# ktncktnc/diffusion-forcing-transformer

Hardware: AMD Instinct MI355X
Metric: denoised latent frames/sec, DFoT RE10K 8f & 200f rollout @1/2/4/8 GPU (higher is better)
Workload: dtype bf16

## Files before the change

### diffusion-forcing-transformer_amd/backbone.py

```python
from __future__ import annotations

import ctypes as C
import math
from typing import Dict, Optional, Sequence, Tuple

import torch
from torch import nn

from . import capi, ops


def _get(cfg, key, default=None):
    if isinstance(cfg, dict):
        return cfg.get(key, default)
    return getattr(cfg, key, default) if not hasattr(cfg, "get") else cfg.get(key, default)


class _Node(nn.Module):
    """Anonymous container so that dotted reference key names map onto a module tree."""


class UViT3DPose(nn.Module):
    def __init__(self, cfg, x_shape: Sequence[int], max_tokens: int, external_cond_dim: int = 0,
                 external_cond_type: str = "action", external_cond_num_classes: Optional[int] = None,
                 use_causal_mask: bool = False, **kwargs):
        super().__init__()
        block_types = list(_get(cfg, "block_types", ["ResBlock", "ResBlock", "TransformerBlock", "TransformerBlock"]))
        if block_types != ["ResBlock", "ResBlock", "TransformerBlock", "TransformerBlock"]:
            raise ValueError(f"unsupported block_types {block_types}")
        if _get(cfg, "pos_emb_type", "rope") != "rope":
            raise ValueError("only pos_emb_type='rope' is supported")
        if not _get(cfg, "use_fourier_noise_embedding", True):
            raise ValueError("only the Fourier noise-level embedding (continuous diffusion) is supported")
        cond = _get(cfg, "conditioning", None)
        cond_dim = _get(cond, "dim", None) if cond is not None else None
        self.cfg = cfg
        self.x_shape = tuple(x_shape)
        self.max_tokens = self.temporal_length = int(max_tokens)
        self.external_cond_dim = int(cond_dim or 180)
        self.use_causal_mask = use_causal_mask
        c = capi.UViTConfig()
        c.channels[:] = list(_get(cfg, "channels"))
        c.emb_channels = int(_get(cfg, "emb_channels"))
        c.num_updown_blocks[:] = list(_get(cfg, "num_updown_blocks"))
        c.num_mid_blocks = int(_get(cfg, "num_mid_blocks"))
        c.num_heads = int(_get(cfg, "num_heads"))
        c.in_channels = int(self.x_shape[0])
        c.resolution = int(self.x_shape[-1])
        c.max_tokens = self.max_tokens
        c.cond_dim = self.external_cond_dim
        c.noise_dim = 256
        c.rope_theta = 10000.0
        c.eps = 1e-6
        if int(_get(cfg, "patch_size", 2)) != 2:
            raise ValueError("only patch_size=2 is supported")
        self._ccfg = c
        self._handle = C.c_void_p()
        capi.check(capi.lib.dfot_uvit_create(C.byref(c), C.byref(self._handle)))
        self._names = []
        self._persistent_buffers = {"noise_level_pos_embedding.timesteps.freqs",
                                    "noise_level_pos_embedding.timesteps.phases"}
        shape = (C.c_int64 * 4)()
        ndim = C.c_int()
        for i in range(capi.lib.dfot_uvit_num_params(self._handle)):
            name = capi.lib.dfot_uvit_param_name(self._handle, i).decode()
            capi.check(capi.lib.dfot_uvit_param_shape(self._handle, i, shape, C.byref(ndim)))
            self._register(name, tuple(shape[k] for k in range(ndim.value)))
            self._names.append(name)
        self._synced: Optional[Tuple] = None
        self._reserved = 0
        self._op_key: Optional[int] = None
        self._cond_key = None
        self._cond_refs = None
        self._cond_gen = None
        self._cond_flag = None
        self.cond_cache_stats = {"builds": 0, "identity_hits": 0, "content_hits": 0}
        self._train_names = None
        self._trainer = None
        self._trainer_sig = None
        self.live_frames = None
        self.fresh_frames = None
        self._fresh_key = None
        self._train_stamp = 0
        self._dropout_generator: Optional[torch.Generator] = None

    def _register(self, name: str, shape: Tuple[int, ...]) -> None:
        *path, leaf = name.split(".")
        node: nn.Module = self
        for part in path:
            if part not in node._modules:
                node.add_module(part, _Node())
            node = node._modules[part]
        t = torch.zeros(shape, dtype=torch.float32)
        if name in self._persistent_buffers:
            node.register_buffer(leaf, t, persistent=True)
        else:
            node.register_parameter(leaf, nn.Parameter(t))

    def _tensors(self) -> Dict[str, torch.Tensor]:
        sd = dict(self.named_parameters())
        sd.update(dict(self.named_buffers()))
        return sd

    def reset_parameters(self, seed: int = 0) -> None:
        g = torch.Generator().manual_seed(seed)
        with torch.no_grad():
            for name, t in self._tensors().items():
                leaf = name.rsplit(".", 1)[-1]
                if leaf == "freqs":
                    t.copy_(2 * math.pi * torch.randn(t.shape, generator=g))
                elif leaf == "phases":
                    t.copy_(2 * math.pi * torch.rand(t.shape, generator=g))
                elif any(s in name for s in (".attn_out.", ".mlp_out.2.", ".out_rest.1.", "project_output")):
                    t.zero_()
                elif leaf == "bias":
                    t.zero_()
                elif t.ndim == 1:
                    t.fill_(1.0)
                else:
                    fan_in = math.prod(t.shape[1:])
                    bound = 1.0 / math.sqrt(fan_in)
                    t.copy_((torch.rand(t.shape, generator=g) * 2 - 1) * bound)

    def _signature(self) -> Tuple:
        return tuple((t.data_ptr(), t._version) for t in self._tensors().values())

    def sync_weights(self, force: bool = False) -> None:
        sig = self._signature()
        if not force and sig == self._synced:
            return
        tensors = self._tensors()
        s = capi.stream_ptr()
        for name in self._names:
            t = tensors[name]
            if not t.is_cuda:
                raise RuntimeError(f"parameter {name} is on {t.device}; move the module to the GPU first")
            src = t.detach().to(torch.float32).contiguous()
            shape = (C.c_int64 * src.ndim)(*src.shape)
            capi.check(capi.lib.dfot_uvit_load_weight(self._handle, name.encode(), capi.ptr(src), shape, src.ndim, s))
        capi.check(capi.lib.dfot_uvit_finalize(self._handle, s))
        self._synced = sig
        self.reserve_generation = getattr(self, "reserve_generation", 0) + 1

    def set_option(self, key: str, value: int) -> None:
        self.reserve_generation = getattr(self, "reserve_generation", 0) + 1
        capi.check(capi.lib.dfot_uvit_set_option(self._handle, key.encode(), int(value)))

    def query(self, key: str) -> float:
        self.sync_weights()
        val = C.c_double()
        capi.check(capi.lib.dfot_uvit_query(self._handle, key.encode(), C.byref(val)))
        return float(val.value)

    def attn_timing(self):
        tot, n = C.c_double(), C.c_int64()
        capi.check(capi.lib.dfot_uvit_attn_timing(self._handle, C.byref(tot), C.byref(n)))
        return tot.value, n.value

    def init_random(self, seed: int = 0, zero_init_scale: float = 0.3) -> None:
        g = torch.Generator().manual_seed(seed)
        with torch.no_grad():
            for name, t in self._tensors().items():
                leaf = name.rsplit(".", 1)[-1]
                if leaf == "freqs":
                    v = 2 * math.pi * torch.randn(t.shape, generator=g)
# ... 89 lines not shown
            out.append(eng.dx_in.to(grad_out.dtype))
        return out

    def _cond_content_equal(self, cond: torch.Tensor, mask: Optional[torch.Tensor]) -> bool:
        if self._cond_key is None or self._cond_refs is None:
            return False
        kept, kept_mask = self._cond_refs
        _, version, shape, synced, mask_key = self._cond_key
        if synced != self._synced or self._cond_gen != self.reserve_generation:
            return False
        if kept._version != version or (kept_mask is not None and kept_mask._version != mask_key[1]):
            return False
        for t in (cond, kept):
            if t.dtype != torch.float32 or not t.is_contiguous():
                return False
        if cond.device != kept.device or tuple(cond.shape) != shape:
            return False
        if (mask is None) != (kept_mask is None):
            return False
        if mask is not None and (mask.dtype != kept_mask.dtype or mask.shape != kept_mask.shape or mask.device != kept_mask.device
                                 or not mask.is_contiguous() or not kept_mask.is_contiguous()):
            return False
        if torch.cuda.is_current_stream_capturing():
            return False
        if self._cond_flag is None or self._cond_flag.device != cond.device:
            self._cond_flag = torch.zeros(1, dtype=torch.int32, device=cond.device)
        flag = self._cond_flag
        flag.zero_()
        s = capi.stream_ptr()
        capi.check(capi.lib.dfot_op_equal_bits(capi.ptr(kept), capi.ptr(cond), cond.numel() * cond.element_size(), capi.ptr(flag), s))
        if mask is not None:
            capi.check(capi.lib.dfot_op_equal_bits(capi.ptr(kept_mask), capi.ptr(mask), mask.numel() * mask.element_size(), capi.ptr(flag), s))
        return int(flag.item()) == 0

    def _forward_impl(self, x: torch.Tensor, noise_levels: torch.Tensor, external_cond: Optional[torch.Tensor] = None,
                      external_cond_mask: Optional[torch.Tensor] = None) -> torch.Tensor:
        assert x.shape[1] == self.temporal_length, (
            f"Temporal length of U-ViT is set to {self.temporal_length}, but input has temporal length {x.shape[1]}.")
        assert external_cond is not None, "External condition (camera pose) is required for U-ViT3DPose model."
        b = x.shape[0]
        if tuple(x.shape[2:]) != self.x_shape:
            raise ValueError(f"x has frame shape {tuple(x.shape[2:])}, expected {self.x_shape}")
        if tuple(external_cond.shape) != (b, self.temporal_length, self.external_cond_dim, *self.x_shape[1:]):
            raise ValueError(f"external_cond has shape {tuple(external_cond.shape)}")
        if external_cond_mask is not None:
            assert external_cond_mask.ndim == 1, "embedding mask should be of shape (B,)"
        if tuple(noise_levels.shape) != (b, self.temporal_length):
            raise ValueError(f"noise_levels has shape {tuple(noise_levels.shape)}, expected {(b, self.temporal_length)}")
        dev = next(self.parameters()).device
        if dev.type != "cuda":
            raise RuntimeError(f"the backbone's parameters are on {dev}; move the module to the GPU first (there is no CPU path)")
        capi.require_device(dev, x=x, noise_levels=noise_levels, external_cond=external_cond, external_cond_mask=external_cond_mask)
        self.sync_weights()
        self.reserve(b)
        xf = x.detach().to(torch.float32).contiguous()
        kf = noise_levels.detach().to(torch.float32).contiguous()
        key = (external_cond.data_ptr(), external_cond._version, tuple(external_cond.shape), self._synced,
               None if external_cond_mask is None else (external_cond_mask.data_ptr(), external_cond_mask._version))
        if key == self._cond_key:
            self.cond_cache_stats["identity_hits"] += 1
        else:
            if self._cond_content_equal(external_cond, external_cond_mask):
                self.cond_cache_stats["content_hits"] += 1
            else:
                cf = external_cond.detach().to(torch.float32).contiguous()
                mf = None if external_cond_mask is None else external_cond_mask.to(torch.uint8).contiguous()
                capi.check(capi.lib.dfot_uvit_set_conditions(self._handle, capi.ptr(cf, torch.float32, "external_cond"),
                                                             capi.ptr(mf, torch.uint8, "external_cond_mask"), b, capi.stream_ptr()))
                self.cond_cache_stats["builds"] += 1
            self._cond_key = key
            self._cond_refs = (external_cond, external_cond_mask)
            self._cond_gen = self.reserve_generation
        out = torch.empty_like(xf)
        live = self.live_frames
        if live is not None:
            if tuple(live.shape) != (b, self.temporal_length) or live.dtype != torch.uint8 or not live.is_contiguous():
                raise ValueError(f"live_frames must be a contiguous uint8 tensor of shape {(b, self.temporal_length)}")
            capi.require_device(dev, live_frames=live)
        fresh = self.fresh_frames
        if fresh is not None:
            if tuple(fresh.shape) != (b, self.temporal_length) or fresh.dtype != torch.uint8 or not fresh.is_contiguous():
                raise ValueError(f"fresh_frames must be a contiguous uint8 tensor of shape {(b, self.temporal_length)}")
            capi.require_device(dev, fresh_frames=fresh)
            if key != self._fresh_key:
                fresh = None
        capi.check(capi.lib.dfot_uvit_forward_cached_masks(self._handle, capi.ptr(xf, torch.float32, "x"),
                                                           capi.ptr(kf, torch.float32, "noise_levels"), capi.ptr(out), b,
                                                           capi.ptr(live, torch.uint8, "live_frames"),
                                                           capi.ptr(fresh, torch.uint8, "fresh_frames"), capi.stream_ptr()))
        self._fresh_key = key
        return out.to(x.dtype)

    def read_tap(self, name: str, channels: int, level: int, batch: int) -> torch.Tensor:
        r = self.x_shape[-1] // 2 // (2 ** level)
        out = torch.empty(batch * self.temporal_length, channels, r, r, device="cuda", dtype=torch.float32)
        capi.check(capi.lib.dfot_uvit_read_tap(self._handle, name.encode(), capi.ptr(out), out.numel(), capi.stream_ptr()))
        return out

    def __del__(self):
        try:
            if getattr(self, "_handle", None) and self._handle.value:
                capi.lib.dfot_uvit_destroy(self._handle)
                self._handle = C.c_void_p()
        except Exception:
            pass
```

### diffusion-forcing-transformer_amd/capi.py

```python
from __future__ import annotations

import ctypes as C
import os

_HERE = os.path.dirname(os.path.abspath(__file__))
LIB_PATH = os.environ.get("DFOT_LIB", os.path.join(_HERE, "libdfot_hip.so"))

OK, ERR_ARG, ERR_SHAPE, ERR_HIP, ERR_STATE, ERR_NAME = range(6)


class DfotError(RuntimeError):
    def __init__(self, code: int, message: str):
        super().__init__(f"libdfot_hip error {code}: {message}")
        self.code = code


class UViTConfig(C.Structure):
    _fields_ = [
        ("channels", C.c_int32 * 4), ("emb_channels", C.c_int32), ("num_updown_blocks", C.c_int32 * 3),
        ("num_mid_blocks", C.c_int32), ("num_heads", C.c_int32), ("in_channels", C.c_int32),
        ("resolution", C.c_int32), ("max_tokens", C.c_int32), ("cond_dim", C.c_int32), ("noise_dim", C.c_int32),
        ("rope_theta", C.c_float), ("eps", C.c_float),
    ]


class UViT3DConfig(C.Structure):
    _fields_ = UViTConfig._fields_ + [("cond_dropout", C.c_int32)]


class DiTConfig(C.Structure):
    _fields_ = [
        ("hidden_size", C.c_int32), ("depth", C.c_int32), ("num_heads", C.c_int32), ("patch_size", C.c_int32),
        ("in_channels", C.c_int32), ("height", C.c_int32), ("width", C.c_int32), ("max_tokens", C.c_int32),
        ("mlp_hidden", C.c_int32), ("noise_dim", C.c_int32), ("timesteps", C.c_int32),
        ("rope_theta", C.c_float), ("eps", C.c_float),
        ("variant", C.c_int32), ("embed_col_dim", C.c_int32), ("num_col_heads", C.c_int32), ("num_row_heads", C.c_int32),
        ("temporal_mlp_hidden", C.c_int32), ("use_bias", C.c_int32),
        ("cond_type", C.c_int32), ("cond_dim", C.c_int32), ("num_classes", C.c_int32), ("cond_dropout", C.c_int32),
        ("use_temporal_rope", C.c_int32),
    ]


class DiTConfigF(DiTConfig):
    _fields_ = [("fourier_noise", C.c_int32)]


class DiT1DConfig(C.Structure):
    _fields_ = [
        ("hidden", C.c_int32), ("depth", C.c_int32), ("heads", C.c_int32), ("mlp_hidden", C.c_int32), ("in_channels", C.c_int32),
        ("tokens_per_frame", C.c_int32), ("max_tokens", C.c_int32), ("timesteps", C.c_int32), ("causal", C.c_int32), ("eps", C.c_float),
    ]


COND_NONE, COND_ACTION, COND_LABEL = 0, 1, 2
ATTN_MAP_OFF, ATTN_MAP_FRAME, ATTN_MAP_FULL = -1, 0, 1


_P, _I, _L, _F = C.c_void_p, C.c_int, C.c_int64, C.c_float
_I32 = C.c_int32


class GemmDesc(C.Structure):
    _fields_ = [
        ("amode", _I32), ("epi", _I32), ("variant", _I32),
        ("A", _P), ("lda", _L), ("W", _P), ("ldw", _L),
        ("M", _I32), ("N", _I32), ("K", _I32), ("H", _I32), ("Wd", _I32), ("Cin", _I32),
        ("live", _P), ("bias", _P), ("bias_rows", _I32),
        ("out_f32", _P), ("out_bf16", _P), ("ldo", _L),
        ("resid", _P), ("resid_bf", _P),
        ("gate", _P), ("gate_index", _P), ("ldg", _L), ("gate_rows", _I32),
        ("act", _I32), ("pre_act", _P), ("raw", _P), ("ldraw", _L), ("tr_rows", _I32),
        ("gn_part", _P), ("gn_rows_per_bt", _I32), ("gn_cpg", _I32),
        ("out2", _P), ("ldo2", _L), ("split", _I32),
        ("q", _P), ("k", _P), ("v", _P),
        ("qw", _P), ("kw", _P), ("rope_cs", _P),
        ("heads", _I32), ("d", _I32), ("ntok", _I32), ("qscale", _F), ("dstride", _I32), ("eps", _F),
        ("ksplit", _I32), ("slice_stride", _L),
    ]


SIGNATURES = {
    "dfot_last_error": (C.c_char_p, []),
    "dfot_version": (_I, []),
    "dfot_uvit_create": (_I, [C.POINTER(UViTConfig), C.POINTER(_P)]),
    "dfot_uvit_destroy": (_I, [_P]),
    "dfot_uvit_num_params": (_I, [_P]),
    "dfot_uvit_param_name": (C.c_char_p, [_P, _I]),
    "dfot_uvit_param_shape": (_I, [_P, _I, C.POINTER(_L), C.POINTER(_I)]),
    "dfot_uvit_load_weight": (_I, [_P, C.c_char_p, _P, C.POINTER(_L), _I, _P]),
    "dfot_uvit_finalize": (_I, [_P, _P]),
    "dfot_uvit_reserve": (_I, [_P, _I]),
    "dfot_uvit_workspace_bytes": (C.c_size_t, [_P]),
    "dfot_uvit_set_option": (_I, [_P, C.c_char_p, _I]),
    "dfot_uvit_query": (_I, [_P, C.c_char_p, C.POINTER(C.c_double)]),
    "dfot_uvit_attn_timing": (_I, [_P, C.POINTER(C.c_double), C.POINTER(_L)]),
    "dfot_uvit_forward": (_I, [_P, _P, _P, _P, _P, _P, _I, _P]),
    "dfot_uvit_set_conditions": (_I, [_P, _P, _P, _I, _P]),
    "dfot_uvit_forward_cached": (_I, [_P, _P, _P, _P, _I, _P]),
    "dfot_uvit_forward_cached_live": (_I, [_P, _P, _P, _P, _I, _P, _P]),
    "dfot_uvit_forward_cached_masks": (_I, [_P, _P, _P, _P, _I, _P, _P, _P]),
    "dfot_uvit_read_tap": (_I, [_P, C.c_char_p, _P, C.c_size_t, _P]),
    "dfot_uvit3d_create": (_I, [C.POINTER(UViT3DConfig), C.POINTER(_P)]),
    "dfot_uvit3d_config_bytes": (_L, []),
    "dfot_uvit3d_forward": (_I, [_P, _P, _P, _P, _P, _P, _I, _P]),
    "dfot_uvit3d_forward_live": (_I, [_P, _P, _P, _P, _P, _P, _I, _P, _P]),
    "dfot_op_gn_film_silu": (_I, [_P, _P, _P, _P, _P, _P, _P, _P, _I, _I, _I, _I, _P]),
    "dfot_op_rms_film": (_I, [_P, _P, _P, _P, _P, _P, _L, _I, _I, _I, _F, _P]),
    "dfot_dit_create": (_I, [C.POINTER(DiTConfig), C.POINTER(_P)]),
    "dfot_dit_create_f": (_I, [C.POINTER(DiTConfigF), C.POINTER(_P)]),
    "dfot_dit_destroy": (_I, [_P]),
    "dfot_dit_num_params": (_I, [_P]),
    "dfot_dit_param_name": (C.c_char_p, [_P, _I]),
    "dfot_dit_param_shape": (_I, [_P, _I, C.POINTER(_L), C.POINTER(_I)]),
    "dfot_dit_load_weight": (_I, [_P, C.c_char_p, _P, C.POINTER(_L), _I, _P]),
    "dfot_dit_finalize": (_I, [_P, _P]),
    "dfot_dit_reserve": (_I, [_P, _I]),
    "dfot_dit_workspace_bytes": (C.c_size_t, [_P]),
    "dfot_dit_set_option": (_I, [_P, C.c_char_p, _I]),
    "dfot_dit_attn_timing": (_I, [_P, C.POINTER(C.c_double), C.POINTER(_L)]),
    "dfot_dit_forward": (_I, [_P, _P, _P, _P, _I, _I, _P]),
    "dfot_dit_forward_cond": (_I, [_P, _P, _P, _P, _P, _P, _P, _I, _I, _P]),
    "dfot_dit_forward_f": (_I, [_P, _P, _P, _P, _P, _P, _P, _I, _I, _P]),
    "dfot_dit_read_tap": (_I, [_P, C.c_char_p, _P, C.c_size_t, _P]),
    "dfot_dit_capture_attention": (_I, [_P, C.POINTER(_I32), _I, _I, C.c_size_t]),
    "dfot_dit_attention_map_shape": (_I, [_P, _I, C.POINTER(_L), C.POINTER(_I)]),
    "dfot_dit_read_attention_map": (_I, [_P, _I, _P, C.c_size_t, _P]),
    "dfot_dit_train_create": (_I, [C.POINTER(DiTConfig), C.POINTER(_P)]),
    "dfot_dit_train_create_f": (_I, [C.POINTER(DiTConfigF), C.POINTER(_P)]),
    "dfot_facmat_train_create": (_I, [C.POINTER(DiTConfigF), C.POINTER(_P)]),
    "dfot_facdit_train_create": (_I, [C.POINTER(DiTConfigF), C.POINTER(_P)]),
    "dfot_dit_train_destroy": (_I, [_P]),
    "dfot_dit_train_num_params": (_I, [_P]),
    "dfot_dit_train_param_name": (C.c_char_p, [_P, _I]),
    "dfot_dit_train_param_shape": (_I, [_P, _I, C.POINTER(_L), C.POINTER(_I)]),
    "dfot_dit_train_param_offset": (_L, [_P, _I]),
    "dfot_dit_train_total_numel": (_L, [_P]),
    "dfot_dit_train_workspace_bytes": (C.c_size_t, [_P]),
    "dfot_dit_train_attach": (_I, [_P, _P, _P]),
    "dfot_dit_train_reserve": (_I, [_P, _I]),
    "dfot_dit_train_sync_weights": (_I, [_P, _P]),
    "dfot_dit_train_forward": (_I, [_P, _P, _P, _P, _I, _I, _P]),
    "dfot_dit_train_forward_cond": (_I, [_P, _P, _P, _P, _P, _P, _P, _I, _I, _P]),
    "dfot_dit_train_load_buffer": (_I, [_P, C.c_char_p, _P, _L, _P]),
    "dfot_dit_train_forward_f": (_I, [_P, _P, _P, _P, _P, _P, _P, _I, _I, _P]),
    "dfot_dit_train_input_grad": (_I, [_P, _P, _P]),
    "dfot_dit_train_backward": (_I, [_P, _P, _P]),
    "dfot_vloss_grad": (_I, [_P] * 7 + [_I, _I, _L, _I, _P]),
    "dfot_sumsq": (_I, [_P, _L, _P, _P]),
    "dfot_adamw_step": (_I, [_P, _P, _P, _P, _L, _F, _F, _F, _F, _F, _I, _P, _F, _P, _F, _P]),
    "dfot_ray_encode": (_I, [_P, _P, _I, _I, _I, _P]),
    "dfot_ray_encode_normalized": (_I, [_P, _P, _I, _I, _I, _P]),
    "dfot_hg_prepare": (_I, [_P, _P, _P, _P, _P, _I, _I, _I, _L, _P]),
    "dfot_ddim_compose": (_I, [_P] * 11 + [_I, _I, _I, _L, _P]),
    "dfot_ddim_compose_tokw": (_I, [_P] * 11 + [_I, _I, _I, _L, _P]),
    "dfot_ddim_noise": (_I, [_P] * 5 + [_I, _I, _I, _L, _I, _P]),
    "dfot_vpred_loss": (_I, [_P] * 9 + [_I, _I, _L, _P]),
    "dfot_vpred_loss_scratch_floats": (_L, [_I, _I, _L]),
    "dfot_vspace_loss": (_I, [_P] * 9 + [_I, _I, _L, _P]),
    "dfot_op_gemm": (_I, [_P, _I, _P, _P, _P, _I, _I, _I, _I, _P]),
    "dfot_op_conv3x3": (_I, [_P, _P, _P, _P, _I, _I, _I, _I, _I, _I, _P]),
    "dfot_op_gemm_ex": (_I, [C.POINTER(GemmDesc), _P]),
    "dfot_op_gemm_desc_bytes": (_L, []),
    "dfot_op_attention": (_I, [_P, _P, _P, _P, _I, _I, _I, _I, _I, _I, _P]),
    "dfot_op_attention_padded": (_I, [_P, _P, _P, _P, _I, _I, _I, _I, _I, _P]),
    "dfot_op_attention_seq64": (_I, [_P, _P, _P, _P, _I, _I, _I, _I, _P]),
    "dfot_op_attention_temporal": (_I, [_P, _P, _P, _P, _I, _I, _I, _I, _I, _I, _P]),
    "dfot_op_attention_temporal_bwd": (_I, [_P, _P, _P, _P, _I, _P, _P, _P, _I, _I, _I, _I, _I, _P]),
    "dfot_op_matrix_attention_rope": (_I, [_P, _P, _P, _I, _I, _I, _I, _I, _I, _F, _P]),
    "dfot_op_matrix_attention_rope_bwd": (_I, [_P, _P, _P, _P, _I, _I, _I, _I, _I, _I, _F, _P]),
    "dfot_op_attention_map_workspace_bytes": (C.c_size_t, [_I, _I, _I, _I, _I]),
    "dfot_op_attention_map": (_I, [_P, _P, _P, _P, C.c_size_t, _I, _I, _I, _I, _I, _I, _P]),
    "dfot_op_attention_temporal_map": (_I, [_P, _P, _P, _P, C.c_size_t, _I, _I, _I, _I, _I, _P]),
    "dfot_op_matrix_attention_map": (_I, [_P, _P, _P, _I, _I, _I, _I, _I, _I, _F, _P]),
    "dfot_op_matrix_attention": (_I, [_P, _P, _I, _I, _I, _I, _I, _I, _F, _P]),
    "dfot_op_facmat_contract": (_I, [_P, _P, _P, _I, _I, _I, _I, _P]),
    "dfot_op_facmat_expand": (_I, [_P, _P, _P, _I, _I, _I, _I, _P]),
    "dfot_op_attention_bwd": (_I, [_P, _P, _P, _P, _P, _I, _P, _P, _P, _I, _I, _I, _I, _P]),
    "dfot_op_conv3x3_bwd": (_I, [_P, _P, _P, _P, _P, _P, _I, _I, _I, _I, _I, _P]),
    "dfot_op_conv3x3_bwd2": (_I, [_P, _P, _P, _P, _P, _P, _P, _I, _I, _I, _I, _I, _P]),
    "dfot_op_gn_silu_bwd": (_I, [_P, _P, _P, _P, _P, _F, _P, _P, _P, _P, _I, _I, _I, _P]),
    "dfot_op_rms_film_bwd": (_I, [_P, _P, _P, _P, _F, _P, _P, _P, _L, _I, _I, _P]),
    "dfot_op_rms_film_bwd_res": (_I, [_P, _P, _P, _P, _F, _P, _P, _P, _P, _P, _L, _I, _P]),
    "dfot_op_qknorm_rope_bwd": (_I, [_P, _I, _P, _P, _P, _P, _P, _P, _F, _P, _I, _P, _P, _L, _I, _I, _I, _P]),
# ... 140 lines not shown
```

### diffusion-forcing-transformer_amd/csrc/gemm.h

```cpp
#pragma once
#include "common.h"

namespace dfot {

enum AMode { A_DENSE = 0, A_CONV3 = 1, A_CONV3T = 2 };
enum Epi { E_F32 = 0, E_BF16 = 1, E_QKV = 2, E_QKV_DIT = 3 };

struct GemmArgs {
  const bf16* A = nullptr;
  long lda = 0;
  const bf16* W = nullptr;
  long ldw = 0;
  int M = 0, N = 0, K = 0;
  int H = 0, Wd = 0, Cin = 0;
  const bf16* zeros = nullptr;
  const uint8_t* live = nullptr;
  int To = 0, Tin = 0, Hin = 0, Win = 0;
  int cs = 1, ct = 1, ckt = 1;
  const float* bias = nullptr;
  float* out_f32 = nullptr;
  bf16* out_bf16 = nullptr;
  long ldo = 0;
  const float* resid = nullptr;
  const bf16* resid_bf = nullptr;
  const float* gate = nullptr;
  const int* gate_index = nullptr;
  long ldg = 0;
  int gate_rows = 0;
  int act = 0;
  bf16* pre_act = nullptr;
  bf16* raw = nullptr;
  long ldraw = 0;
  int bias_rows = 0;
  int tr_rows = 0;
  float* gn_part = nullptr;
  int gn_rows_per_bt = 0;
  int gn_cpg = 0;
  bf16* out2 = nullptr;
  long ldo2 = 0;
  int split = 0;
  bf16 *q = nullptr, *k = nullptr, *v = nullptr;
  const float *qw = nullptr, *kw = nullptr, *rope_cs = nullptr;
  int heads = 0, d = 0, ntok = 0;
  float qscale = 1.f;
  int dstride = 0;
  float eps = 1e-6f;
  int xcd = 1;
  int persist = 0;
  int ksplit = 1;
  long slice_stride = 0;
};

enum GemmVariant {
  GEMM_REGS_128 = 0,
  GEMM_DMA_128 = 1,
  GEMM_DMA_256x256 = 4,
  GEMM_DMA_512x128 = 6,
  GEMM_DMA_128_KS2 = 8,
  GEMM_DMA_256x192 = 9,
  GEMM_DMA_128x192 = 10,
  GEMM_DMA3_256x144 = 14,
  GEMM_AUTO = -1
};
int gemm_pick_variant(int amode, int m, int n, int k, bool plain_f32 = false);
int launch_gemm(int amode, int epi, int variant, const GemmArgs& g, hipStream_t stream);

}
```

### diffusion-forcing-transformer_amd/csrc/gemm.hip

```cpp
#include "gemm.h"
#include "dfot_hip.h"

namespace dfot {

constexpr int BK = 64;
constexpr int wave_cols(int bn) { return bn % 64 == 0 ? 64 : 48; }
constexpr int tile_threads(int bm, int bn, int wtm, int ks) { return (bm / wtm) * (bn / wave_cols(bn)) * 64 * ks; }
constexpr int EP_LD = 68;

template <int N>
__device__ __forceinline__ void wait_all_but() {
  static_assert(N == 2 || N == 4 || N == 6 || N == 8 || N == 12, "unexpected load count");
  if constexpr (N == 2) asm volatile("s_waitcnt vmcnt(2)\n\ts_barrier" ::: "memory");
  if constexpr (N == 4) asm volatile("s_waitcnt vmcnt(4)\n\ts_barrier" ::: "memory");
  if constexpr (N == 6) asm volatile("s_waitcnt vmcnt(6)\n\ts_barrier" ::: "memory");
  if constexpr (N == 8) asm volatile("s_waitcnt vmcnt(8)\n\ts_barrier" ::: "memory");
  if constexpr (N == 12) asm volatile("s_waitcnt vmcnt(12)\n\ts_barrier" ::: "memory");
}

__device__ __forceinline__ void wait_all_but_n(int n) {
  switch (n) {
    case 1: asm volatile("s_waitcnt vmcnt(1)\n\ts_barrier" ::: "memory"); break;
    case 2: asm volatile("s_waitcnt vmcnt(2)\n\ts_barrier" ::: "memory"); break;
    case 3: asm volatile("s_waitcnt vmcnt(3)\n\ts_barrier" ::: "memory"); break;
// ... 741 lines not shown
  constexpr int lds = stage_lds > ep_lds ? stage_lds : ep_lds;
  const int ksplit = (EPI == E_F32 && (AMODE == A_DENSE || g.slice_stride > 0) && g.ksplit > 1) ? g.ksplit : 1;
  const int tiles = (g.M / BM_T) * ((g.N + BN_T - 1) / BN_T) * ksplit;
  GemmArgs ga = g;
  ga.xcd = 1;
  ga.persist = 1;
  constexpr bool kPersistOK = KS == 1 && nthreads <= 768;
  if constexpr (kPersistOK) {
    if (ga.persist > 0 && ksplit == 1) {
      const int resident = 256 * (lds <= 80 * 1024 ? 2 : 1);
      if (tiles > resident) {
        auto kp = gemm_kernel_persistent<BM_T, BN_T, WTM, NST, AMODE, EPI, DMA, KS, BKT>;
        static bool pattr_set = false;
        if (!pattr_set) {
          DFOT_CHECK_HIP(hipFuncSetAttribute(reinterpret_cast<const void*>(kp), hipFuncAttributeMaxDynamicSharedMemorySize, lds));
          pattr_set = true;
        }
        hipLaunchKernelGGL(kp, dim3(resident), dim3(nthreads), lds, stream, ga, tiles);
        DFOT_CHECK_HIP(hipGetLastError());
        return DFOT_OK;
      }
    }
  }
  auto kern = gemm_kernel<BM_T, BN_T, WTM, NST, AMODE, EPI, DMA, KS, BKT>;
  static bool attr_set = false;
  if (!attr_set) {
    DFOT_CHECK_HIP(hipFuncSetAttribute(reinterpret_cast<const void*>(kern), hipFuncAttributeMaxDynamicSharedMemorySize, lds));
    attr_set = true;
  }
  hipLaunchKernelGGL(kern, dim3(tiles), dim3(nthreads), lds, stream, ga);
  DFOT_CHECK_HIP(hipGetLastError());
  return DFOT_OK;
}

template <int AMODE, int EPI>
static int launch_v(int variant, const GemmArgs& g, hipStream_t s) {
  switch (variant) {
    case GEMM_REGS_128:
      if constexpr (AMODE == A_CONV3T) break;
      else return launch_t<128, 128, 64, 2, AMODE, EPI, false>(g, s);
    case GEMM_DMA_128: return launch_t<128, 128, 64, 2, AMODE, EPI, true>(g, s);
    case GEMM_DMA_256x256: return launch_t<256, 256, 64, 2, AMODE, EPI, true>(g, s);
    case GEMM_DMA_512x128: return launch_t<512, 128, 64, 2, AMODE, EPI, true>(g, s);
    case GEMM_DMA_256x192:
      if constexpr (AMODE != A_DENSE) break;
      else return launch_t<256, 192, 64, 2, AMODE, EPI, true>(g, s);
    case GEMM_DMA3_256x144:
      if constexpr ((EPI != E_F32 && !(EPI == E_BF16 && AMODE == A_DENSE)) || AMODE == A_CONV3T) break;
      else {
        if (g.gn_part) break;
        return launch_t<256, 144, 64, 3, AMODE, EPI, true>(g, s);
      }
    case GEMM_DMA_128x192:
      if constexpr (AMODE != A_DENSE || EPI == E_QKV) break;
      else return launch_t<128, 192, 64, 2, AMODE, EPI, true>(g, s);
    case GEMM_DMA_128_KS2:
      if constexpr (EPI == E_QKV) break;
      else return launch_t<128, 128, 64, 2, AMODE, EPI, true, 2>(g, s);
  }
  set_error("gemm: unknown variant %d", variant);
  return DFOT_ERR_ARG;
}

int gemm_pick_variant(int amode, int m, int n, int k, bool plain_f32) {
  const long tiles = (long)(m / 256) * ((n + 255) / 256);
  if (m % 256 == 0 && n >= 192 && amode == A_DENSE) {
    auto util = [&](int bn) {
      const long t = (long)(m / 256) * ((n + bn - 1) / bn);
      return (double)m * n / ((double)((t + 255) / 256) * 256 * 256 * bn);
    };
    if (plain_f32 && n % 144 == 0 && k >= 2304 && (long)(m / 256) * (n / 144) >= 256 && util(144) > 1.1 * util(192) && util(144) > 1.1 * util(256))
      return GEMM_DMA3_256x144;
    if (util(192) > 1.05 * util(256) && (long)(m / 256) * ((n + 191) / 192) >= 160) return GEMM_DMA_256x192;
  }
  if (m % 256 == 0 && n >= 192 && tiles >= 160) return GEMM_DMA_256x256;
  if (m % 512 == 0 && n <= 128 && m / 512 >= 256) return GEMM_DMA_512x128;
  const long tiles128 = (long)(m / 128) * ((n + 127) / 128);
  if (tiles128 <= 256 && k >= 2048) return GEMM_DMA_128_KS2;
  return GEMM_DMA_128;
}

int launch_gemm(int amode, int epi, int variant, const GemmArgs& g, hipStream_t stream) {
  DFOT_REQUIRE(g.A && g.W, DFOT_ERR_ARG, "gemm: null operand");
  if (variant == GEMM_AUTO) variant = gemm_pick_variant(amode, g.M, g.N, g.K, epi == E_F32 && !g.gn_part);
  if (variant == GEMM_DMA_128_KS2 && epi == E_QKV) variant = GEMM_DMA_128;
  if (variant == GEMM_DMA_128x192 && epi == E_QKV) variant = GEMM_DMA_128;
  if (variant == GEMM_DMA_256x192 && epi == E_QKV && g.d != 64) variant = GEMM_DMA_256x256;
  const int bm = variant == GEMM_DMA_512x128 ? 512 : (variant == GEMM_DMA_256x256 || variant == GEMM_DMA_256x192 || variant == GEMM_DMA3_256x144) ? 256 : 128;
  DFOT_REQUIRE(g.M > 0 && g.M % bm == 0, DFOT_ERR_SHAPE, "gemm: M=%d must be a positive multiple of %d", g.M, bm);
  DFOT_REQUIRE(g.K > 0 && g.K % BK == 0, DFOT_ERR_SHAPE, "gemm: K=%d must be a positive multiple of %d", g.K, BK);
  DFOT_REQUIRE(g.N > 0 && g.N % (epi == E_F32 ? 4 : 8) == 0, DFOT_ERR_SHAPE, "gemm: N=%d must be a multiple of %d", g.N, epi == E_F32 ? 4 : 8);
  DFOT_REQUIRE((epi == E_QKV || epi == E_QKV_DIT || g.ldo % (epi == E_F32 ? 4 : 8) == 0) && (epi != E_QKV || (g.ldo2 % 8 == 0 && g.split % 64 == 0)),
               DFOT_ERR_SHAPE, "gemm: output row strides must be multiples of %d", epi == E_F32 ? 4 : 8);
  DFOT_REQUIRE(g.ldw == 0 || (amode == A_DENSE && g.ldw >= g.K && g.ldw % 8 == 0), DFOT_ERR_SHAPE, "gemm: ldw=%ld must be >= K and a multiple of 8 (dense A only)", g.ldw);
  if (amode == A_CONV3) {
    DFOT_REQUIRE(g.Cin % BK == 0 && g.K == 9 * g.Cin, DFOT_ERR_SHAPE, "conv3x3: Cin=%d must be a multiple of %d", g.Cin, BK);
    DFOT_REQUIRE(g.zeros != nullptr, DFOT_ERR_ARG, "conv3x3: zero page missing");
    DFOT_REQUIRE(g.H > 0 && g.Wd > 0 && g.M % (g.H * g.Wd) == 0, DFOT_ERR_SHAPE, "conv3x3: M=%d not a whole number of %dx%d images", g.M, g.H, g.Wd);
    DFOT_REQUIRE(!g.live || (g.H * g.Wd) % bm == 0, DFOT_ERR_SHAPE, "conv3x3: live-image flags need whole %d-row tiles per %dx%d image", bm, g.H, g.Wd);
  }
  if (amode == A_CONV3T) {
    DFOT_REQUIRE(epi == E_F32 && g.ksplit <= 1 && !g.live && !g.gate && !g.bias_rows, DFOT_ERR_ARG, "conv3t: plain fp32 epilogue only");
    DFOT_REQUIRE(g.Cin % BK == 0 && (g.ckt == 1 || g.ckt == 3) && g.K == g.ckt * 9 * g.Cin && (g.cs == 1 || g.cs == 2) && (g.ct == 1 || g.ct == 2),
                 DFOT_ERR_SHAPE, "conv3t: Cin=%d (multiple of %d), kt=%d in {1,3}, K=%d = kt*9*Cin, strides s=%d t=%d in {1,2}", g.Cin, BK, g.ckt, g.K,
                 g.cs, g.ct);
    DFOT_REQUIRE(g.zeros != nullptr, DFOT_ERR_ARG, "conv3t: zero page missing");
    DFOT_REQUIRE(g.H > 0 && g.Wd > 0 && g.To > 0 && g.Hin == g.cs * g.H && g.Win == g.cs * g.Wd && g.Tin >= 1 && g.ct * (g.To - 1) <= g.Tin - 1 &&
                     g.To == (g.Tin - 1) / g.ct + 1,
                 DFOT_ERR_SHAPE, "conv3t: input %dx%dx%d, output %dx%dx%d do not match strides s=%d t=%d", g.Tin, g.Hin, g.Win, g.To, g.H, g.Wd, g.cs, g.ct);
    DFOT_REQUIRE(g.M % (g.To * g.H * g.Wd) == 0, DFOT_ERR_SHAPE, "conv3t: M=%d not a whole number of %dx%dx%d videos", g.M, g.To, g.H, g.Wd);
    DFOT_REQUIRE((long)g.Tin * g.Hin * g.Win * g.Cin < (1L << 31), DFOT_ERR_SHAPE, "conv3t: one input video must hold < 2^31 elements");
  }
  if (epi == E_QKV) {
    DFOT_REQUIRE(g.q && g.k && g.v && g.qw && g.kw && g.rope_cs && (g.out2 || g.N == g.split), DFOT_ERR_ARG, "qkv epilogue: null pointer");
    DFOT_REQUIRE(!g.raw || (g.ldraw >= g.N && g.ldraw % 8 == 0), DFOT_ERR_SHAPE, "qkv epilogue: raw copy needs ldraw >= N, a multiple of 8");
    DFOT_REQUIRE((g.d == 64 || g.d == 128) && g.heads > 0 && g.split == 3 * g.heads * g.d && g.ntok > 0 && g.M % g.ntok == 0,
                 DFOT_ERR_SHAPE, "qkv epilogue: heads=%d d=%d split=%d ntok=%d M=%d", g.heads, g.d, g.split, g.ntok, g.M);
  }
  if (epi == E_QKV_DIT) {
    DFOT_REQUIRE(g.q && g.k && g.v, DFOT_ERR_ARG, "dit qkv epilogue: null pointer");
    DFOT_REQUIRE(g.d > 0 && g.d % 8 == 0 && g.dstride >= g.d && g.dstride % 8 == 0 && g.heads > 0 && g.N == 3 * g.heads * g.d &&
                     g.ntok > 0 && g.M % g.ntok == 0,
                 DFOT_ERR_SHAPE, "dit qkv epilogue: heads=%d d=%d dstride=%d ntok=%d M=%d N=%d", g.heads, g.d, g.dstride, g.ntok, g.M, g.N);
  }
  if (g.gate) {
    DFOT_REQUIRE(epi == E_F32 && g.gate_rows > 0 && g.M % g.gate_rows == 0 && g.ldg % 4 == 0, DFOT_ERR_SHAPE,
                 "gemm: gate needs the fp32 epilogue, gate_rows dividing M and ldg %% 4 == 0");
  }
  if (g.ksplit > 1 && g.slice_stride > 0)
    DFOT_REQUIRE(!g.bias && !g.resid, DFOT_ERR_ARG, "gemm: split-K into partial outputs takes no bias / residual");
  if (g.ksplit > 1)
    DFOT_REQUIRE(epi == E_F32 && (amode == A_DENSE || g.slice_stride > 0) && !g.bias_rows && (!g.resid || g.resid == g.out_f32) && !g.gate &&
                     !g.gn_part && g.K / BK >= 2 * g.ksplit, DFOT_ERR_ARG,
                 "gemm: split-K over workgroups needs the fp32 epilogue with an in-place residual (or none), no gate, and K >= %d", 2 * g.ksplit * BK);
  if (g.bias_rows) DFOT_REQUIRE((epi == E_F32 || epi == E_BF16) && g.bias, DFOT_ERR_ARG, "gemm: 2-D bias needs a plain epilogue");
  if (g.resid_bf)
    DFOT_REQUIRE(epi == E_BF16 && (amode == A_CONV3 || variant == GEMM_DMA3_256x144) && !g.resid, DFOT_ERR_ARG,
                 "gemm: a bf16 residual needs the bf16 epilogue of a convolution or of the 256x144 ring");
  if (g.tr_rows) {
    DFOT_REQUIRE(epi == E_BF16 && !g.bias && !g.act && !g.gn_part && g.tr_rows % 4 == 0 && g.M % g.tr_rows == 0 && amode == A_DENSE,
                 DFOT_ERR_ARG, "gemm: transposed store needs the plain bf16 epilogue and tr_rows %% 4 == 0 dividing M");
  }
  if (g.gn_part) {
    DFOT_REQUIRE(epi != E_QKV && epi != E_QKV_DIT && (g.gn_cpg == 4 || g.gn_cpg == 8) && g.N == 32 * g.gn_cpg && g.gn_rows_per_bt % 64 == 0 &&
                     g.gn_rows_per_bt % bm == 0,
                 DFOT_ERR_SHAPE, "gemm: fused GroupNorm statistics need N = 32 groups of 4 or 8 channels and whole images per tile");
  }
  if (amode == A_DENSE) {
    switch (epi) {
      case E_F32: return launch_v<A_DENSE, E_F32>(variant, g, stream);
      case E_BF16: return launch_v<A_DENSE, E_BF16>(variant, g, stream);
      case E_QKV: return launch_v<A_DENSE, E_QKV>(variant, g, stream);
      case E_QKV_DIT: return launch_v<A_DENSE, E_QKV_DIT>(variant, g, stream);
    }
  } else if (amode == A_CONV3) {
    switch (epi) {
      case E_F32: return launch_v<A_CONV3, E_F32>(variant, g, stream);
      case E_BF16: return launch_v<A_CONV3, E_BF16>(variant, g, stream);
    }
  } else if (amode == A_CONV3T && epi == E_F32) {
    return launch_v<A_CONV3T, E_F32>(variant, g, stream);
  }
  set_error("gemm: unsupported mode/epilogue combination %d/%d", amode, epi);
  return DFOT_ERR_ARG;
}

}
// ... 1 lines not shown
```

### diffusion-forcing-transformer_amd/csrc/kernels.h

```cpp
#pragma once
#include "common.h"

namespace dfot {

int launch_noise_emb(const float* k, const float* freqs, const float* phases, const float* w1, const float* b1,
                     const float* w2, const float* b2, float* hidden, float* out, int bt, int ndim, int e, hipStream_t s);
int launch_uvit3d_emb(const float* k, const float* freqs, const float* phases, const float* w1, const float* b1, const float* w2,
                      const float* b2, const float* cond, const uint8_t* cond_mask, const float* a_w1, const float* a_b1,
                      const float* a_w2, const float* a_b2, float* out, int bt, int ndim, int cdim, int e, int tokens, hipStream_t s);
int launch_embed_input(const float* x, const float* w, const float* b, float* out, int bt, int res, int cin, int c0,
                       hipStream_t s);
int launch_cond_repack(const float* cond, bf16* a, int bt, int res, int cdim, int kpad, hipStream_t s);
int launch_emb_pyramid(const bf16* emb0, bf16* emb1, bf16* emb2, bf16* emb3, int bt, int r0, int e, hipStream_t s);
int launch_project_output(const float* x0, const float* w, const float* b, float* out, int bt, int res, int c0, int cout,
                          hipStream_t s, const uint8_t* live = nullptr);
int launch_gn_partial_f32(const float* x, float* partial, int bt, int pixels, int c, hipStream_t s);
int launch_gn_partial_bf16(const bf16* x, float* partial, int bt, int pixels, int c, hipStream_t s);
int launch_gn_finalize(const float* partial, float* stats, int bt, int nblk, int pixels, int c, float eps, hipStream_t s);
int gn_partial_blocks(int pixels);
int launch_gn_apply_silu(const float* x, const float* stats, const float* gamma, const float* beta, bf16* out, int bt,
                         int pixels, int c, hipStream_t s, const uint8_t* live = nullptr);
struct FilmChunk {
  const bf16* w;
  const float* b;
  long out_off;
  int rows;
};
int launch_film_vec(const FilmChunk* table, int chunks, const float* nemb, float* sv, int bt, int e, hipStream_t s);
int launch_gn_film_silu(const bf16* h, const float* stats, const float* gamma, const float* beta, const bf16* fcache,
                        const float* sv, const uint8_t* cond_mask, bf16* out, int bt, int pixels, int c, int tokens,
                        hipStream_t s, const uint8_t* live = nullptr);
struct RmsPending {
  void* x;
  const float* bias;
  const float* s0;
  const float* s1;
  const float* s2;
};
int launch_rms_film(const float* x, const float* w, const bf16* fcache, const float* sv, const uint8_t* cond_mask, bf16* out,
                    long m, int c, int rows_per_bt, int tokens, float eps, hipStream_t s, const RmsPending* pend = nullptr);
int launch_rms_film_bf16(const bf16* x, const float* w, const bf16* fcache, const float* sv, const uint8_t* cond_mask, bf16* out,
                         long m, int c, int rows_per_bt, int tokens, float eps, hipStream_t s, const RmsPending* pend = nullptr);

int launch_pool2_bf16(const float* x, bf16* out, int bt, int h, int w, int c, hipStream_t s);
int launch_pool2_bf16_bf16in(const bf16* x, bf16* out, int bt, int h, int w, int c, hipStream_t s);
int launch_sub_bf16_bf16in(const bf16* a, const float* b, bf16* out, long n, hipStream_t s, const uint8_t* live = nullptr, long frame_elems = 0);
int launch_upsample_add_bf16(const float* t, const bf16* skip, bf16* out, int bt, int h, int w, int c, hipStream_t s, const uint8_t* live = nullptr);
int launch_gn_apply_silu_bf16in(const bf16* x, const float* stats, const float* gamma, const float* beta, bf16* out, int bt, int pixels, int c,
                                hipStream_t s, const uint8_t* live = nullptr);
int launch_embed_input_bf16(const float* x, const float* w, const float* b, bf16* out, int bt, int res, int cin, int c0, hipStream_t s);
int launch_project_output_bf16(const bf16* x0, const float* w, const float* b, float* out, int bt, int res, int c0, int cout, hipStream_t s,
                               const uint8_t* live = nullptr);
int launch_sub_bf16(const float* a, const float* b, bf16* out, long n, hipStream_t s, const uint8_t* live = nullptr, long frame_elems = 0);
int launch_upsample_add(const float* t, const float* skip, float* out, int bt, int h, int w, int c, hipStream_t s, const uint8_t* live = nullptr);
int launch_ray_encode(const float* poses, float* out, int b, int t, int res, int normalized, hipStream_t s);
int launch_hg_prepare(const float* x, const float* noise, const float* qa, const float* qb, float* x_in, int batch,
                      int nfe, int tokens, long f, hipStream_t s);
int launch_ddim_compose(const float* x, const float* x_in, const float* v, const float* sa, const float* s1,
                        const float* an, const float* cn, const float* keep, const float* weight, const uint8_t* gen,
                        float* x_next, int batch, int nfe, int tokens, long f, bool weight_per_token, hipStream_t s);
int launch_ddim_noise(const float* noise, const float* sigma, const float* weight, const uint8_t* gen, float* x_next, int batch, int nfe,
                      int tokens, long f, bool weight_per_token, hipStream_t s);
int vloss_chunks(long f);
int launch_vloss(const float* x, const float* noise, const float* v, const float* a, const float* sg, const float* w,
                 float* x_pred, float* partial, float* loss, int batch, int tokens, long f, bool vspace, hipStream_t s);
int launch_wgrad_nt(const bf16* a, long lda, const bf16* b, long ldb, float* out, int m, int n, long rows, int slices, hipStream_t s, int img_h = 0,
                    int img_w = 0, int sdy = 0, int sdx = 0, int all_taps = 0);
struct WgradPlan {
  int form, slices;
};
WgradPlan wgrad_plan(int m, int n, long rows, long max_slices);
int launch_wgrad_conv_taps(const bf16* dy, const bf16* x, float* out, int co, int ci, long pix, int slices, int img_h, int img_w, hipStream_t s);
int wgrad_conv_tiles(int co, int ci, int* target);
int launch_wgrad_nt_plan(const bf16* a, long lda, const bf16* b, long ldb, float* out, int m, int n, long rows, WgradPlan plan, hipStream_t s);
int launch_vloss_grad(const float* x, const float* noise, const float* v, const float* a, const float* sg, const float* coef, float* dv,
                      int batch, int tokens, long f, bool vspace, hipStream_t s);
int launch_sumsq(const float* x, long n, float* out, hipStream_t s);
int launch_adamw(float* p, const float* g, float* m, float* v, long n, float lr, float b1, float b2, float eps, float wd, int step,
                 const float* sumsq, float max_norm, float* ema, float ema_decay, hipStream_t s);
int launch_f32_to_bf16(const float* src, bf16* dst, long n, hipStream_t s);
int launch_bf16_to_f32(const bf16* src, float* dst, long n, hipStream_t s);
int launch_equal_bits(const void* a, const void* b, long bytes, int* differs, hipStream_t s);
int launch_pack_rows(const float* src, bf16* dst, const int* map, int rows, int k, int kpad, long ldd, int col0,
                     hipStream_t s);
int launch_pack_conv3(const float* src, bf16* dst, int co, int ci, hipStream_t s);
int launch_gather_f32(const float* src, float* dst, const int* map, int n, hipStream_t s);
int launch_nhwc_to_nchw(const float* src, float* dst, int bt, int p, int c, hipStream_t s);
int launch_bf16_nhwc_to_nchw(const bf16* src, float* dst, int bt, int p, int c, hipStream_t s);

struct AttnScratch {
  float* p = nullptr;
  size_t bytes = 0;
};
int launch_attention(const bf16* q, const bf16* k, const bf16* v, bf16* o, long ldo, int batch, int heads, int n, int d,
                     int variant, hipStream_t stream, AttnScratch* scratch = nullptr);
int launch_attention_v3(const bf16* q, const bf16* k, const bf16* v, bf16* o, long ldo, int batch, int heads, int n, bool nomax,
                        hipStream_t stream, AttnScratch* scratch = nullptr);
bool attention_v5_applies(int n, int d, float score_bound);
int launch_attention_v5(const bf16* q, const bf16* k, const bf16* v, bf16* o, long ldo, int batch, int heads, int n, hipStream_t stream,
                        AttnScratch* scratch = nullptr, float* lse = nullptr);
bool attention_ks_applies(int batch, int heads, int n, int d);
size_t attention_ks_scratch_bytes(int batch, int heads, int n, int d);
int launch_attention_ks(const bf16* q, const bf16* k, const bf16* v, bf16* o, long ldo, int batch, int heads, int n, hipStream_t stream,
                        AttnScratch* scratch = nullptr);
int attention_dstride(int d);
int launch_attention_padded(const bf16* q, const bf16* k, const bf16* v, bf16* o, long ldo, int batch, int heads, int n, int d,
                            hipStream_t stream, float* lse = nullptr);
int launch_attention_seq64(const bf16* q, const bf16* k, const bf16* v, bf16* o, long ldo, int nseq, int heads, int d, hipStream_t stream);
int launch_attention_frame_causal(const bf16* q, const bf16* k, const bf16* v, bf16* o, long ldo, int batch, int heads, int n, int frame_len,
                                  int d, hipStream_t stream);
int launch_attention_temporal(const bf16* q, const bf16* k, const bf16* v, bf16* o, long ldo, int batch, int tokens, int patches, int heads,
                              int d, hipStream_t s);
int launch_attention_temporal_bwd(const bf16* q, const bf16* k, const bf16* v, const bf16* d_o, long ldo, bf16* dq, bf16* dk, bf16* dv,
                                  int batch, int tokens, int patches, int heads, int d, hipStream_t s);
int launch_matrix_attn_rope(const bf16* z, bf16* o, const float* rope_cs, int batch, int L, int E, int h, int cc, int rr, float scale,
                            hipStream_t s);
int launch_matrix_attn_rope_bwd(const bf16* z, const bf16* d_o, const float* rope_cs, bf16* dz, int batch, int L, int E, int h, int cc, int rr,
                                float scale, hipStream_t s);
int launch_facmat_contract(const bf16* m, const bf16* u, bf16* w, int frames, int P, int h, int E, hipStream_t s);
int launch_facmat_expand(const bf16* o, const bf16* u, bf16* sp, int frames, int P, int h, int E, hipStream_t s);
size_t attention_map_part_floats(int batch, int heads, int n, int tokens);
int launch_attention_map(const bf16* q, const bf16* k, float* out, float* part, bool full, int batch, int heads, int n, int tokens, int d,
                         hipStream_t s);
size_t attention_temporal_map_part_floats(int batch, int heads, int tokens, int patches);
int launch_attention_temporal_map(const bf16* q, const bf16* k, float* out, float* part, int batch, int tokens, int patches, int heads, int d,
                                  hipStream_t s);
int launch_matrix_attn_map(const bf16* z, const float* rope_cs, float* out, int batch, int L, int E, int h, int cc, int rr, float scale,
                           hipStream_t s);
struct AttnSplit {
  int tiles, full, rem, nsplit;
  int slots;
};
AttnSplit attn_plan_split(int batch, int heads, int n, int qrows, int wgs_per_cu);
size_t attn_partial_bytes(const AttnSplit& sp, int qrows, int dcols);
size_t attention_scratch_bytes(int batch, int heads, int n, int d);
int attn_partials(const AttnSplit& sp, int qrows, int dcols, float** po, float** pml, AttnScratch* scratch);
int attn_launch_merge(const AttnSplit& sp, int qrows, int dcols, const float* po, const float* pml, bf16* o, long ldo, int n, int heads,
                      hipStream_t stream, float* lse = nullptr);
int launch_attention_bwd_delta(const bf16* o, const bf16* d_o, long ldo, float* delta, int batch, int heads, int n, int d, hipStream_t s);
int launch_attention_bwd(const bf16* q, const bf16* k, const bf16* v, const bf16* d_o, long ldo, const float* l2, const float* delta,
                         bf16* dq, bf16* dk, bf16* dv, int batch, int heads, int n, int d, hipStream_t s);

}
```

### diffusion-forcing-transformer_amd/csrc/kernels.hip

```cpp
#include "kernels.h"
#include "dfot_hip.h"

namespace dfot {

typedef __attribute__((ext_vector_type(4))) float float4v;
typedef __attribute__((ext_vector_type(2))) float float2v;

__device__ __forceinline__ float wave_sum(float v) {
#pragma unroll
  for (int o = 32; o > 0; o >>= 1) v += __shfl_xor(v, o);
  return v;
}

template <bool FOURIER>
__global__ __launch_bounds__(256) void noise_mlp_kernel(const float* __restrict__ in, const float* __restrict__ freqs,
                                                        const float* __restrict__ phases, const float* __restrict__ w,
                                                        const float* __restrict__ b, float* __restrict__ out, int kdim,
                                                        int e) {
  const int lane = threadIdx.x & 63, wave = threadIdx.x >> 6;
  const int row = blockIdx.x * 4 + wave;
  const int bt = blockIdx.y;
  if (row >= e) return;
  float acc = 0.f;
  for (int i = lane; i < kdim; i += 64) {
// ... 1441 lines not shown
  if (!part) DFOT_CHECK_HIP(hipMalloc(&part, SUMSQ_BLOCKS * sizeof(float)));
  hipLaunchKernelGGL(sumsq_partial_kernel, dim3(SUMSQ_BLOCKS), dim3(256), 0, s, x, n, part);
  hipLaunchKernelGGL(sumsq_final_kernel, dim3(1), dim3(256), 0, s, part, out);
  DFOT_CHECK_HIP(hipGetLastError());
  return DFOT_OK;
}

__global__ void adamw_kernel(float* __restrict__ p, const float* __restrict__ g, float* __restrict__ m, float* __restrict__ v, long n,
                             float lr, float b1, float b2, float eps, float wd, float c1, float c2, const float* __restrict__ sumsq,
                             float max_norm, float* __restrict__ ema, float ema_decay) {
  const long i = (long)blockIdx.x * blockDim.x + threadIdx.x;
  if (i >= n) return;
  float clip = 1.f;
  if (sumsq) clip = fminf(1.f, max_norm / (sqrtf(*sumsq) + 1e-6f));
  const float gv = g[i] * clip;
  const float mv = b1 * m[i] + (1.f - b1) * gv;
  const float vv = b2 * v[i] + (1.f - b2) * gv * gv;
  m[i] = mv;
  v[i] = vv;
  const float pv = p[i] * (1.f - lr * wd);
  const float pn = pv - (lr / c1) * mv / (sqrtf(vv) / sqrtf(c2) + eps);
  p[i] = pn;
  if (ema) ema[i] = ema_decay * ema[i] + (1.f - ema_decay) * pn;
}
int launch_adamw(float* p, const float* g, float* m, float* v, long n, float lr, float b1, float b2, float eps, float wd, int step,
                 const float* sumsq, float max_norm, float* ema, float ema_decay, hipStream_t s) {
  DFOT_REQUIRE(step >= 1, DFOT_ERR_ARG, "adamw: step counts from 1");
  const float c1 = (float)(1.0 - pow((double)b1, (double)step)), c2 = (float)(1.0 - pow((double)b2, (double)step));
  hipLaunchKernelGGL(adamw_kernel, dim3(cdiv(n, 256)), dim3(256), 0, s, p, g, m, v, n, lr, b1, b2, eps, wd, c1, c2, sumsq, max_norm, ema, ema_decay);
  DFOT_CHECK_HIP(hipGetLastError());
  return DFOT_OK;
}

typedef __attribute__((ext_vector_type(4))) unsigned int uint4v;
__device__ __forceinline__ unsigned int bits_differ(uint4v x, uint4v y) {
  const uint4v d = x ^ y;
  return d[0] | d[1] | d[2] | d[3];
}
__device__ __forceinline__ unsigned int bits_differ(unsigned int x, unsigned int y) { return x ^ y; }
__device__ __forceinline__ unsigned int bits_differ(uint8_t x, uint8_t y) { return (unsigned int)(x ^ y); }

constexpr int EQ_BLOCK = 256, EQ_MAX_GRID = 2048;

template <typename T>
__global__ __launch_bounds__(EQ_BLOCK) void equal_bits_kernel(const T* __restrict__ a, const T* __restrict__ b, long n, int rest,
                                                              int* __restrict__ differs) {
  const long stride = (long)gridDim.x * EQ_BLOCK;
  long i = (long)blockIdx.x * EQ_BLOCK + threadIdx.x;
  unsigned int acc = 0;
  for (; i + 3 * stride < n; i += 4 * stride) {
    const T a0 = a[i], a1 = a[i + stride], a2 = a[i + 2 * stride], a3 = a[i + 3 * stride];
    const T b0 = b[i], b1 = b[i + stride], b2 = b[i + 2 * stride], b3 = b[i + 3 * stride];
    acc |= bits_differ(a0, b0) | bits_differ(a1, b1) | bits_differ(a2, b2) | bits_differ(a3, b3);
  }
  for (; i < n; i += stride) acc |= bits_differ(a[i], b[i]);
  if (blockIdx.x == 0 && (int)threadIdx.x < rest) {
    const uint8_t* ta = reinterpret_cast<const uint8_t*>(a + n);
    const uint8_t* tb = reinterpret_cast<const uint8_t*>(b + n);
    acc |= bits_differ(ta[threadIdx.x], tb[threadIdx.x]);
  }
  if (acc) *differs = 1;
}

template <typename T>
static int launch_equal_bits_t(const void* a, const void* b, long bytes, int* differs, hipStream_t s) {
  const long n = bytes / (long)sizeof(T);
  const int rest = (int)(bytes - n * (long)sizeof(T));
  const int grid = n ? (int)(cdiv(n, EQ_BLOCK) < EQ_MAX_GRID ? cdiv(n, EQ_BLOCK) : EQ_MAX_GRID) : 1;
  hipLaunchKernelGGL(equal_bits_kernel<T>, dim3(grid), dim3(EQ_BLOCK), 0, s, (const T*)a, (const T*)b, n, rest, differs);
  DFOT_CHECK_HIP(hipGetLastError());
  return DFOT_OK;
}

int launch_equal_bits(const void* a, const void* b, long bytes, int* differs, hipStream_t s) {
  DFOT_REQUIRE(differs && ((uintptr_t)differs & 3) == 0, DFOT_ERR_ARG, "equal_bits: the flag is null or not 4-byte aligned");
  DFOT_REQUIRE(bytes >= 0, DFOT_ERR_ARG, "equal_bits: negative length %ld", bytes);
  if (bytes == 0) return DFOT_OK;
  DFOT_REQUIRE(a && b, DFOT_ERR_ARG, "equal_bits: null buffer");
  const uintptr_t al = (uintptr_t)a | (uintptr_t)b;
  if ((al & 15) == 0) return launch_equal_bits_t<uint4v>(a, b, bytes, differs, s);
  if ((al & 3) == 0) return launch_equal_bits_t<unsigned int>(a, b, bytes, differs, s);
  return launch_equal_bits_t<uint8_t>(a, b, bytes, differs, s);
}
}

extern "C" int dfot_op_equal_bits(const void* a, const void* b, int64_t bytes, int32_t* differs, void* stream) {
  return dfot::launch_equal_bits(a, b, (long)bytes, differs, (hipStream_t)stream);
}
```

### diffusion-forcing-transformer_amd/csrc/uvit.hip

```cpp
#include <algorithm>
#include <cmath>
#include <cstdarg>
#include <cstdlib>
#include <cstring>
#include <functional>
#include <map>
#include <string>
#include <vector>

#include "dfot_hip.h"
#include "gemm.h"
#include "kernels.h"

namespace dfot {

static thread_local char g_err[1024] = "";
void set_error(const char* fmt, ...) {
  va_list ap;
  va_start(ap, fmt);
  vsnprintf(g_err, sizeof(g_err), fmt, ap);
  va_end(ap);
}
const char* get_error() { return g_err; }

// ... 256 lines not shown
    bf16* pw = h->pose_w;
    const int k = c.cond_dim * 4, kp = h->kpose;
    add_param(h, "external_cond_embedding.patch_embedder.proj.weight", {e, c.cond_dim, 2, 2},
              [=](const float* src, hipStream_t s) { return launch_pack_rows(src, pw, nullptr, e, k, kp, kp, 0, s); });
    if ((rc = add_f32(h, "external_cond_embedding.patch_embedder.proj.bias", {e}, &h->pose_b))) return rc;
  }
  if ((rc = add_f32(h, "embed_input.proj.weight", {h->ch[0], c.in_channels, 2, 2}, &h->ein_w))) return rc;
  if ((rc = add_f32(h, "embed_input.proj.bias", {h->ch[0]}, &h->ein_b))) return rc;
  if ((rc = add_f32(h, "project_output.proj.weight", {h->ch[0], c.in_channels, 2, 2}, &h->pout_w))) return rc;
  if ((rc = add_f32(h, "project_output.proj.bias", {c.in_channels}, &h->pout_b))) return rc;

  for (int l = 0; l < 3; ++l) {
    const int n = c.num_updown_blocks[l];
    const std::string pre = "down_blocks." + std::to_string(l) + ".";
    if (l < 2) {
      h->down_res[l].resize(n);
      for (int i = 0; i < n; ++i)
        if ((rc = add_res_block(h, pre + std::to_string(i), h->ch[l], &h->down_res[l][i]))) return rc;
    } else {
      h->down_tr.resize(n);
      for (int i = 0; i < n; ++i)
        if ((rc = add_tr_block(h, pre + std::to_string(i), l, &h->down_tr[i]))) return rc;
    }
    if ((rc = add_conv(h, pre + std::to_string(n) + ".conv", h->ch[l], h->ch[l + 1], &h->down_conv[l]))) return rc;
  }
  auto add_mid = [&]() -> int {
    h->mid_tr.resize(c.num_mid_blocks);
    for (int i = 0; i < c.num_mid_blocks; ++i)
      if ((rc = add_tr_block(h, "mid_blocks." + std::to_string(i), 3, &h->mid_tr[i]))) return rc;
    return DFOT_OK;
  };
  if (!h->posefree && (rc = add_mid())) return rc;
  for (int j = 0; j < 3; ++j) {
    const int l = 2 - j;
    const int n = c.num_updown_blocks[l];
    const std::string pre = "up_blocks." + std::to_string(j) + ".";
    if ((rc = add_conv(h, pre + "0.conv", h->ch[l + 1], h->ch[l], &h->up_conv[l]))) return rc;
    if (l < 2) {
      h->up_res[l].resize(n);
      for (int i = 0; i < n; ++i)
        if ((rc = add_res_block(h, pre + std::to_string(i + 1), h->ch[l], &h->up_res[l][i]))) return rc;
    } else {
      h->up_tr.resize(n);
      for (int i = 0; i < n; ++i)
        if ((rc = add_tr_block(h, pre + std::to_string(i + 1), l, &h->up_tr[i]))) return rc;
    }
  }
  if (h->posefree && (rc = add_mid())) return rc;
  return DFOT_OK;
}

static int build_rope(dfot_uvit_s* h, int lvl) {
  const int d = h->ch[lvl] / h->heads, half = d / 2;
  const int q = half / 3, rem = half % 3;
  int parts[3] = {q, q, q};
  if (rem == 1) parts[0] = q + 1;
  if (rem == 2) parts[1] = parts[2] = q + 1;
  const int rr = h->r[lvl], n = h->T * rr * rr;
  std::vector<float> cs((size_t)n * half * 2);
  for (int tok = 0; tok < n; ++tok) {
    const int pos[3] = {tok / (rr * rr), (tok / rr) % rr, tok % rr};
    int pair = 0;
    for (int ax = 0; ax < 3; ++ax) {
      const int dim = 2 * parts[ax];
      for (int j = 0; j < parts[ax]; ++j, ++pair) {
        const float inv = 1.0f / powf(h->cfg.rope_theta, (float)(2 * j) / (float)dim);
        const float ang = (float)pos[ax] * inv;
        cs[((size_t)tok * half + pair) * 2 + 0] = cosf(ang);
        cs[((size_t)tok * half + pair) * 2 + 1] = sinf(ang);
      }
    }
  }
  int rc = dev_alloc(h, &h->rope_cs[lvl], cs.size());
  if (rc) return rc;
  DFOT_CHECK_HIP(hipMemcpy(h->rope_cs[lvl], cs.data(), cs.size() * sizeof(float), hipMemcpyHostToDevice));
  return DFOT_OK;
}

__global__ void add_vec_kernel(const float* a, const float* b, float* o, int n) {
  const int i = blockIdx.x * blockDim.x + threadIdx.x;
  if (i < n) o[i] = a[i] + b[i];
}

static int run_res_block(dfot_uvit_s* h, const ResW& w, int lvl, int bt, hipStream_t s, const uint8_t* live = nullptr) {
  const int c = w.c, rr = h->r[lvl], pix = rr * rr;
  const int m = bt * pix;
  const int slots = pix / 64;
  bf16* xb = h->XB[lvl];
  int rc = 0;
  if (!h->xin_bf[lvl]) {
    if ((rc = launch_f32_to_bf16(h->xin[lvl], xb, (long)m * c, s))) return rc;
    h->xin_bf[lvl] = true;
  }
  if (h->gn1_nblk == 0) {
    if ((rc = launch_gn_partial_bf16(xb, h->gn_partial, bt, pix, c, s))) return rc;
    h->gn1_nblk = gn_partial_blocks(pix);
  }
  if ((rc = launch_gn_finalize(h->gn_partial, h->gn_stats, bt, h->gn1_nblk, pix, c, h->cfg.eps, s))) return rc;
  h->gn1_nblk = 0;
  if ((rc = launch_gn_apply_silu_bf16in(xb, h->gn_stats, w.g1, w.be1, h->s1, bt, pix, c, s, live))) return rc;
  GemmArgs g;
  g.A = h->s1; g.W = w.w1; g.M = m; g.N = c; g.K = 9 * c; g.H = rr; g.Wd = rr; g.Cin = c; g.zeros = h->zeros;
  g.bias = w.bias1; g.out_bf16 = h->hbf; g.ldo = c; g.live = live;
  g.gn_part = h->gn_partial2; g.gn_rows_per_bt = pix; g.gn_cpg = c / 32;
  if ((rc = launch_gemm(A_CONV3, E_BF16, h->gemm_variant, g, s))) return rc;
  if ((rc = launch_gn_finalize(h->gn_partial2, h->gn_stats, bt, slots, pix, c, h->cfg.eps, s))) return rc;
  if ((rc = launch_gn_film_silu(h->hbf, h->gn_stats, w.g2, w.be2, w.fcache, h->sv + w.sv_off,
                                h->have_mask ? h->cond_mask : nullptr, h->s1, bt, pix, c, h->T, s, live)))
    return rc;
  GemmArgs o;
  o.A = h->s1; o.W = w.w2; o.M = m; o.N = c; o.K = 9 * c; o.H = rr; o.Wd = rr; o.Cin = c; o.zeros = h->zeros;
  o.bias = w.bias2; o.out_bf16 = xb; o.ldo = c; o.live = live;
  o.resid_bf = xb;
  o.gn_part = h->gn_partial; o.gn_rows_per_bt = pix; o.gn_cpg = c / 32;
  if ((rc = launch_gemm(A_CONV3, E_BF16, h->gemm_variant, o, s))) return rc;
  h->xin_bf[lvl] = true;
  h->gn1_nblk = slots;
  return DFOT_OK;
}

__global__ void out_reduce_kernel(bf16* x, const float* __restrict__ bias, const float* __restrict__ s0, const float* __restrict__ s1,
                                  const float* __restrict__ s2, long total4, int cq) {
  typedef __attribute__((ext_vector_type(4))) float f4;
  const long i = (long)blockIdx.x * blockDim.x + threadIdx.x;
  if (i >= total4) return;
  f4 b = reinterpret_cast<const f4*>(bias)[i % cq] + reinterpret_cast<const f4*>(s0)[i] + reinterpret_cast<const f4*>(s1)[i];
  if (s2) b += reinterpret_cast<const f4*>(s2)[i];
  const bf16x4 xv = reinterpret_cast<const bf16x4*>(x)[i];
  reinterpret_cast<bf16x4*>(x)[i] = bf16x4{f2bf(bf2f(xv[0]) + b[0]), f2bf(bf2f(xv[1]) + b[1]), f2bf(bf2f(xv[2]) + b[2]), f2bf(bf2f(xv[3]) + b[3])};
}
__global__ void add_f32_into_bf16_kernel(bf16* x, const float* __restrict__ y, long total4) {
  typedef __attribute__((ext_vector_type(4))) float f4;
  const long i = (long)blockIdx.x * blockDim.x + threadIdx.x;
  if (i >= total4) return;
  const f4 b = reinterpret_cast<const f4*>(y)[i];
  const bf16x4 xv = reinterpret_cast<const bf16x4*>(x)[i];
  reinterpret_cast<bf16x4*>(x)[i] = bf16x4{f2bf(bf2f(xv[0]) + b[0]), f2bf(bf2f(xv[1]) + b[1]), f2bf(bf2f(xv[2]) + b[2]), f2bf(bf2f(xv[3]) + b[3])};
}

static void swap_out_part(dfot_uvit_s* h) { h->pend_part = h->out_part; }

static int flush_pending(dfot_uvit_s* h, hipStream_t s) {
  if (!h->pend_bias) return DFOT_OK;
  const long total4 = h->pend_m * h->pend_c / 4;
  hipLaunchKernelGGL(out_reduce_kernel, dim3(cdiv(total4, 256)), dim3(256), 0, s, h->XB[h->pend_lvl], h->pend_bias, h->pend_part,
                     h->pend_part + h->pend_m * h->pend_c, h->pend_slices == 3 ? h->pend_part + 2 * h->pend_m * h->pend_c : nullptr, total4,
                     h->pend_c / 4);
  h->pend_bias = nullptr;
  DFOT_CHECK_HIP(hipGetLastError());
  return DFOT_OK;
}

static int run_tr_block(dfot_uvit_s* h, const TrW& w, int lvl, int batch, hipStream_t s) {
  const int c = w.c, rr = h->r[lvl], n = h->T * rr * rr, d = c / h->heads;
  const int m = batch * n;
  bf16* xb = h->XB[lvl];
  int rc = 0;
  if (h->pend_bias && (h->pend_lvl != lvl || h->pend_m != m || h->pend_c != c) && (rc = flush_pending(h, s))) return rc;
  if (!h->xin_bf[lvl]) {
    if ((rc = launch_f32_to_bf16(h->xin[lvl], xb, (long)m * c, s))) return rc;
    h->xin_bf[lvl] = true;
  }
  RmsPending pend{xb, h->pend_bias, h->pend_part, h->pend_part + (long)m * c, h->pend_slices == 3 ? h->pend_part + 2L * m * c : nullptr};
  if ((rc = launch_rms_film_bf16(xb, w.nw, w.fcache, h->sv + w.sv_off, h->have_mask ? h->cond_mask : nullptr, h->s1, m, c, rr * rr, h->T,
                                 h->cfg.eps, s, h->pend_bias ? &pend : nullptr)))
    return rc;
  h->pend_bias = nullptr;
  GemmArgs p;
  p.A = h->s1; p.lda = c; p.W = w.w_fused; p.M = m; p.N = 7 * c; p.K = c; p.bias = w.b_fused;
  p.out2 = h->cat + c; p.ldo2 = 5 * c; p.split = 3 * c;
  p.q = h->q; p.k = h->k; p.v = h->v; p.qw = w.qw; p.kw = w.kw; p.rope_cs = h->rope_cs[lvl]; p.heads = h->heads; p.d = d;
  p.ntok = n; p.qscale = 1.4426950408889634f / sqrtf((float)d); p.eps = h->cfg.eps;
  if ((rc = launch_gemm(A_DENSE, E_QKV, h->gemm_variant, p, s))) return rc;
  const bool timed = h->time_attn && lvl == 2 && h->ev_used < h->ev_start.size();
  if (timed) DFOT_CHECK_HIP(hipEventRecord(h->ev_start[h->ev_used], s));
  int av = h->attn_variant;
  if (av == 2 && d == 64 && n % 256 == 0) av = (attention_v5_applies(n, d, w.score_bound) && !h->attn_force_safe) ? 14 : 5;
  if ((rc = launch_attention(h->q, h->k, h->v, h->cat, 5 * c, batch, h->heads, n, d, av, s, &h->attn_scratch))) return rc;
  if (timed) DFOT_CHECK_HIP(hipEventRecord(h->ev_stop[h->ev_used++], s));
  GemmArgs o;
  o.A = h->cat; o.lda = 5 * c; o.W = w.w_out; o.M = m; o.N = c; o.K = 5 * c; o.bias = w.b_out; o.ldo = c;
  if (h->gemm_variant == GEMM_AUTO && h->out_part && (size_t)2 * m * c <= h->out_part_elems && m % 256 == 0 && c % 144 == 0 &&
      (long)(m / 256) * (c / 144) * 2 <= 256 && (5 * c / 64) >= 8) {
    GemmArgs p2 = o;
    p2.bias = nullptr; p2.out_f32 = h->out_part; p2.ksplit = 2; p2.slice_stride = (long)m * c;
    if ((rc = launch_gemm(A_DENSE, E_F32, GEMM_DMA3_256x144, p2, s))) return rc;
    h->pend_bias = w.b_out;
    h->pend_lvl = lvl; h->pend_m = m; h->pend_c = c; h->pend_slices = 2;
    swap_out_part(h);
    return DFOT_OK;
  }
  if (h->gemm_variant == GEMM_AUTO && c % 144 == 0 && m % 256 == 0 && (long)(m / 256) * ((c + 191) / 192) < 256 &&
      (long)(m / 256) * (c / 144) >= 200 && (long)(m / 256) * (c / 144) <= 256) {
    o.out_bf16 = xb;
    o.resid_bf = xb;
    return launch_gemm(A_DENSE, E_BF16, GEMM_DMA3_256x144, o, s);
  }
  o.out_f32 = h->X[lvl];
  if ((rc = launch_gemm(A_DENSE, E_F32, h->gemm_variant, o, s))) return rc;
  hipLaunchKernelGGL(add_f32_into_bf16_kernel, dim3(cdiv((long)m * c / 4, 256)), dim3(256), 0, s, xb, h->X[lvl], (long)m * c / 4);
  DFOT_CHECK_HIP(hipGetLastError());
  return DFOT_OK;
}


__global__ void slab_reduce_kernel(float* __restrict__ out, const float* __restrict__ bias, const float* __restrict__ slabs, int nslab, long stride4,
                                   long total4, int cq, const uint8_t* __restrict__ live, unsigned img4) {
  typedef __attribute__((ext_vector_type(4))) float f4;
  const long i = (long)blockIdx.x * blockDim.x + threadIdx.x;
  if (i >= total4) return;
  if (live && !live[(unsigned)i / img4]) return;
  f4 v = reinterpret_cast<const f4*>(bias)[i % cq];
  for (int sl = 0; sl < nslab; ++sl) v += reinterpret_cast<const f4*>(slabs)[sl * stride4 + i];
  reinterpret_cast<f4*>(out)[i] = v;
}

static int conv_between_levels(dfot_uvit_s* h, GemmArgs g, hipStream_t s) {
  const long px = (long)g.H * g.Wd;
  if (h->gemm_variant == GEMM_AUTO && h->out_part && !g.gn_part && g.M % 256 == 0 && px % 256 == 0 && (g.N % 144 == 0 || g.N == 256) &&
      (long)g.M * g.N < (1L << 31)) {
    const int bn = g.N % 144 == 0 ? 144 : 256;
    const int variant = bn == 144 ? GEMM_DMA3_256x144 : GEMM_DMA_256x256;
    const int tiles = (g.M / 256) * (g.N / bn);
    int ks = 1;
    while (tiles * ks * 2 <= 256 && g.K / 64 / (ks * 2) >= 16) ks *= 2;
    if (tiles * ks >= 192 && tiles * ks <= 256) {
      if (ks == 1) return launch_gemm(A_CONV3, E_F32, variant, g, s);
      if ((size_t)ks * g.M * g.N <= h->out_part_elems) {
        GemmArgs p = g;
        float* out = g.out_f32;
        const float* bias = g.bias;
        p.bias = nullptr; p.resid = nullptr; p.out_f32 = h->out_part; p.ksplit = ks; p.slice_stride = (long)g.M * g.N;
        int rc = launch_gemm(A_CONV3, E_F32, variant, p, s);
        if (rc) return rc;
        const long total4 = (long)g.M * g.N / 4;
        hipLaunchKernelGGL(slab_reduce_kernel, dim3(cdiv(total4, 256)), dim3(256), 0, s, out, bias, h->out_part, ks, total4, total4, g.N / 4, g.live,
                           (unsigned)(px * g.N / 4));
        DFOT_CHECK_HIP(hipGetLastError());
        return DFOT_OK;
      }
    }
  }
  return launch_gemm(A_CONV3, E_F32, h->gemm_variant, g, s);
}

static int run_down(dfot_uvit_s* h, int l, int bt, hipStream_t s, const uint8_t* live = nullptr) {
  const int rr = h->r[l], cin = h->ch[l], cout = h->ch[l + 1];
  int rc = 0;
  if ((rc = h->xin_bf[l] ? launch_pool2_bf16_bf16in(h->XB[l], h->s1, bt, rr, rr, cin, s) : launch_pool2_bf16(h->xin[l], h->s1, bt, rr, rr, cin, s)))
    return rc;
  GemmArgs g;
  g.A = h->s1; g.W = h->down_conv[l].w; g.M = bt * (rr / 2) * (rr / 2); g.N = cout; g.K = 9 * cin; g.H = rr / 2; g.Wd = rr / 2;
  g.Cin = cin; g.zeros = h->zeros; g.bias = h->down_conv[l].b; g.out_f32 = h->HSA[l]; g.ldo = cout;
  g.live = live;
  const bool next_is_res = l + 1 < 2;
  if (next_is_res) {
    g.gn_part = h->gn_partial; g.gn_rows_per_bt = (rr / 2) * (rr / 2); g.gn_cpg = cout / 32;
  }
  if ((rc = conv_between_levels(h, g, s))) return rc;
  h->gn1_nblk = next_is_res ? g.gn_rows_per_bt / 64 : 0;
  h->xin[l + 1] = h->HSA[l];
  h->xin_bf[l + 1] = false;
  return DFOT_OK;
}

static int run_up(dfot_uvit_s* h, int l, int bt, hipStream_t s, const uint8_t* live = nullptr) {
  const int rr = h->r[l + 1], cin = h->ch[l + 1], cout = h->ch[l];
  const long n_in = (long)bt * rr * rr * cin;
  int rc = 0;
  if ((rc = h->xin_bf[l + 1] ? launch_sub_bf16_bf16in(h->XB[l + 1], h->HSA[l], h->s1, n_in, s, live, (long)rr * rr * cin)
                             : launch_sub_bf16(h->xin[l + 1], h->HSA[l], h->s1, n_in, s, live, (long)rr * rr * cin)))
    return rc;
  GemmArgs g;
  g.A = h->s1; g.W = h->up_conv[l].w; g.M = bt * rr * rr; g.N = cout; g.K = 9 * cin; g.H = rr; g.Wd = rr; g.Cin = cin;
  g.zeros = h->zeros; g.bias = h->up_conv[l].b; g.out_f32 = h->tmp; g.ldo = cout;
  if (live && (rr * rr) % 256 == 0 && h->gemm_variant == GEMM_AUTO) g.live = live;
  if ((rc = conv_between_levels(h, g, s))) return rc;
  h->gn1_nblk = 0;
  if (!h->xin_bf[l]) {
    set_error("run_up: level %d stream is not in its bf16 buffer", l);
    return DFOT_ERR_STATE;
  }
  return launch_upsample_add_bf16(h->tmp, h->XB[l], h->XB[l], bt, rr, rr, cout, s, live);
}

}

static int forward_from_emb(dfot_uvit_s* h, const float* x, float* out, int batch, const uint8_t* live_frames, const uint8_t* fresh_frames,
                            hipStream_t s);

extern "C" {

const char* dfot_last_error(void) { return get_error(); }
int dfot_version(void) { return 1; }

int dfot_uvit_create(const dfot_uvit_config* cfg, dfot_uvit_t* out) {
  DFOT_REQUIRE(cfg && out, DFOT_ERR_ARG, "dfot_uvit_create: null argument");
  DFOT_REQUIRE(cfg->resolution % 16 == 0 && cfg->resolution >= 32, DFOT_ERR_SHAPE, "resolution %d must be a multiple of 16", cfg->resolution);
  DFOT_REQUIRE(cfg->emb_channels % 64 == 0, DFOT_ERR_SHAPE, "emb_channels %d must be a multiple of 64", cfg->emb_channels);
  DFOT_REQUIRE(cfg->in_channels <= 3 && cfg->cond_dim % 20 == 0, DFOT_ERR_SHAPE, "in_channels %d / cond_dim %d unsupported", cfg->in_channels, cfg->cond_dim);
  for (int l = 0; l < 4; ++l)
    DFOT_REQUIRE(cfg->channels[l] % 64 == 0, DFOT_ERR_SHAPE, "channels[%d]=%d must be a multiple of 64", l, cfg->channels[l]);
  DFOT_REQUIRE(cfg->channels[0] % 128 == 0 && cfg->channels[1] % 128 == 0, DFOT_ERR_SHAPE, "ResBlock channels must be multiples of 128");
  for (int l = 2; l < 4; ++l) {
    const int d = cfg->channels[l] / cfg->num_heads;
    DFOT_REQUIRE(d * cfg->num_heads == cfg->channels[l] && (d == 64 || d == 128), DFOT_ERR_SHAPE,
                 "level %d head dim %d must be 64 or 128", l, d);
  }
  const int r3 = cfg->resolution / 16;
  DFOT_REQUIRE((cfg->max_tokens * r3 * r3) % 128 == 0, DFOT_ERR_SHAPE, "tokens at the coarsest level (%d) must be a multiple of 128", cfg->max_tokens * r3 * r3);
  auto* h = new dfot_uvit_s();
  h->cfg = *cfg;
  int rc = build(h);
  if (rc) {
    dfot_uvit_destroy(h);
    return rc;
  }
  *out = h;
  return DFOT_OK;
}

int dfot_uvit_destroy(dfot_uvit_t h) {
  if (!h) return DFOT_OK;
  for (void* p : h->owned) (void)hipFree(p);
  for (void* p : h->ws_owned) (void)hipFree(p);
  for (hipEvent_t e : h->ev_start) (void)hipEventDestroy(e);
  for (hipEvent_t e : h->ev_stop) (void)hipEventDestroy(e);
  delete h;
  return DFOT_OK;
}

int dfot_uvit3d_create(const dfot_uvit3d_config* cfg, dfot_uvit_t* out) {
  DFOT_REQUIRE(cfg && out, DFOT_ERR_ARG, "dfot_uvit3d_create: null argument");
  DFOT_REQUIRE(cfg->resolution % 16 == 0 && cfg->resolution >= 32, DFOT_ERR_SHAPE, "resolution %d must be a multiple of 16", cfg->resolution);
  DFOT_REQUIRE(cfg->emb_channels % 64 == 0 && cfg->emb_channels <= 1024, DFOT_ERR_SHAPE,
               "emb_channels %d must be a multiple of 64 and at most 1024", cfg->emb_channels);
  DFOT_REQUIRE(cfg->in_channels >= 1 && cfg->in_channels <= 3, DFOT_ERR_SHAPE, "in_channels %d unsupported (1 .. 3)", cfg->in_channels);
  DFOT_REQUIRE(cfg->cond_dim >= 0 && cfg->cond_dim <= 1024, DFOT_ERR_SHAPE, "cond_dim %d unsupported: the action embedding takes 0 (none) .. 1024 values", cfg->cond_dim);
  DFOT_REQUIRE(cfg->noise_dim > 0 && cfg->noise_dim <= 1024, DFOT_ERR_SHAPE, "noise_dim %d must be 1 .. 1024", cfg->noise_dim);
  for (int l = 0; l < 4; ++l)
    DFOT_REQUIRE(cfg->channels[l] > 0 && cfg->channels[l] % 64 == 0, DFOT_ERR_SHAPE, "channels[%d]=%d must be a multiple of 64", l, cfg->channels[l]);
  DFOT_REQUIRE(cfg->channels[0] % 128 == 0 && cfg->channels[1] % 128 == 0, DFOT_ERR_SHAPE, "ResBlock channels must be multiples of 128");
  DFOT_REQUIRE(cfg->num_heads > 0 && cfg->max_tokens > 0 && cfg->num_mid_blocks >= 0, DFOT_ERR_SHAPE, "num_heads / max_tokens must be positive");
  for (int l = 2; l < 4; ++l) {
    const int d = cfg->channels[l] / cfg->num_heads;
    DFOT_REQUIRE(d * cfg->num_heads == cfg->channels[l] && (d == 64 || d == 128), DFOT_ERR_SHAPE,
                 "level %d head dim %d must be 64 or 128 (channels %d / num_heads %d)", l, d, cfg->channels[l], cfg->num_heads);
  }
  const int r3 = cfg->resolution / 16;
  DFOT_REQUIRE((cfg->max_tokens * r3 * r3) % 128 == 0, DFOT_ERR_SHAPE, "tokens at the coarsest level (%d) must be a multiple of 128", cfg->max_tokens * r3 * r3);
  auto* h = new dfot_uvit_s();
  dfot_uvit_config& c = h->cfg;
  for (int l = 0; l < 4; ++l) c.channels[l] = cfg->channels[l];
  for (int l = 0; l < 3; ++l) c.num_updown_blocks[l] = cfg->num_updown_blocks[l];
  c.emb_channels = cfg->emb_channels; c.num_mid_blocks = cfg->num_mid_blocks; c.num_heads = cfg->num_heads;
  c.in_channels = cfg->in_channels; c.resolution = cfg->resolution; c.max_tokens = cfg->max_tokens;
  c.cond_dim = 0;
  c.noise_dim = cfg->noise_dim; c.rope_theta = cfg->rope_theta; c.eps = cfg->eps;
  h->posefree = true;
  h->act_dim = cfg->cond_dim;
  h->act_dropout = cfg->cond_dim > 0 && cfg->cond_dropout != 0;
  int rc = build(h);
  if (rc) {
    dfot_uvit_destroy(h);
    return rc;
  }
  *out = h;
  return DFOT_OK;
}
int64_t dfot_uvit3d_config_bytes(void) { return (int64_t)sizeof(dfot_uvit3d_config); }

int dfot_uvit_num_params(dfot_uvit_t h) { return h ? (int)h->params.size() : 0; }
// ... 173 lines not shown
    h->ev_used = 0;
    while ((int)h->ev_start.size() < value) {
      hipEvent_t a, b;
      DFOT_CHECK_HIP(hipEventCreate(&a));
      DFOT_CHECK_HIP(hipEventCreate(&b));
      h->ev_start.push_back(a);
      h->ev_stop.push_back(b);
    }
  }
  else {
    set_error("set_option: unknown key '%s'", key);
    return DFOT_ERR_ARG;
  }
  return DFOT_OK;
}

int dfot_uvit_query(dfot_uvit_t h, const char* key, double* value) {
  DFOT_REQUIRE(h && key && value, DFOT_ERR_ARG, "query: null argument");
  DFOT_REQUIRE(h->finalized, DFOT_ERR_STATE, "query: weights not finalized");
  float bound = 0.f;
  for (const TrW& w : h->down_tr) bound = fmaxf(bound, w.score_bound);
  for (const TrW& w : h->up_tr) bound = fmaxf(bound, w.score_bound);
  if (!strcmp(key, "score_bound_l2")) *value = bound;
  else if (!strcmp(key, "attn_kernel_l2")) *value = (bound < 64.0f && !h->attn_force_safe) ? 14 : 5;
  else if (!strcmp(key, "cond_builds")) *value = (double)h->cond_builds;
  else {
    set_error("query: unknown key '%s'", key);
    return DFOT_ERR_ARG;
  }
  return DFOT_OK;
}

int dfot_uvit_set_conditions(dfot_uvit_t h, const float* external_cond, const uint8_t* external_cond_mask, int batch,
                             void* stream) {
  DFOT_REQUIRE(h, DFOT_ERR_ARG, "set_conditions: null handle");
  DFOT_REQUIRE(!h->posefree, DFOT_ERR_STATE, "set_conditions: a pose-free handle (dfot_uvit3d_create) has no pose caches; call dfot_uvit3d_forward");
  DFOT_REQUIRE(external_cond != nullptr, DFOT_ERR_ARG, "External condition (camera pose) is required for U-ViT3DPose model.");
  DFOT_REQUIRE(h->finalized, DFOT_ERR_STATE, "set_conditions: weights not finalized");
  DFOT_REQUIRE(batch > 0 && batch <= h->max_batch, DFOT_ERR_STATE, "set_conditions: batch %d exceeds reserved %d", batch, h->max_batch);
  hipStream_t s = (hipStream_t)stream;
  const dfot_uvit_config& c = h->cfg;
  const int bt = batch * h->T, e = h->E;
  int rc = 0;
  h->cond_batch = 0;
  ++h->cond_builds;
  if ((rc = launch_cond_repack(external_cond, h->acond, bt, c.resolution, c.cond_dim, h->kpose, s))) return rc;
  {
    GemmArgs g;
    g.A = h->acond; g.lda = h->kpose; g.W = h->pose_w; g.M = bt * h->r[0] * h->r[0]; g.N = e; g.K = h->kpose;
    g.bias = h->pose_b; g.out_bf16 = h->emb[0]; g.ldo = e;
    if ((rc = launch_gemm(A_DENSE, E_BF16, h->gemm_variant, g, s))) return rc;
  }
  if ((rc = launch_emb_pyramid(h->emb[0], h->emb[1], h->emb[2], h->emb[3], bt, h->r[0], e, s))) return rc;
  auto fill = [&](bf16* fcache, const bf16* wf, int cc, int lvl) -> int {
    GemmArgs g;
    g.A = h->emb[lvl]; g.lda = e; g.W = wf; g.M = bt * h->r[lvl] * h->r[lvl]; g.N = 2 * cc; g.K = e;
    g.out_bf16 = fcache; g.ldo = 2 * cc;
    return launch_gemm(A_DENSE, E_BF16, h->gemm_variant, g, s);
  };
  for (int l = 0; l < 2; ++l) {
    for (ResW& w : h->down_res[l]) if ((rc = fill(w.fcache, w.w_film, w.c, l))) return rc;
    for (ResW& w : h->up_res[l]) if ((rc = fill(w.fcache, w.w_film, w.c, l))) return rc;
  }
  for (TrW& w : h->down_tr) if ((rc = fill(w.fcache, w.w_film, w.c, 2))) return rc;
  for (TrW& w : h->up_tr) if ((rc = fill(w.fcache, w.w_film, w.c, 2))) return rc;
  for (TrW& w : h->mid_tr) if ((rc = fill(w.fcache, w.w_film, w.c, 3))) return rc;
  h->have_mask = external_cond_mask != nullptr;
  if (h->have_mask) DFOT_CHECK_HIP(hipMemcpyAsync(h->cond_mask, external_cond_mask, batch, hipMemcpyDeviceToDevice, s));
  h->cond_batch = batch;
  return DFOT_OK;
}

int dfot_uvit_forward_cached(dfot_uvit_t h, const float* x, const float* noise_levels, float* out, int batch, void* stream) {
  return dfot_uvit_forward_cached_live(h, x, noise_levels, out, batch, nullptr, stream);
}

int dfot_uvit_forward_cached_live(dfot_uvit_t h, const float* x, const float* noise_levels, float* out, int batch, const uint8_t* live_frames,
                                  void* stream) {
  return dfot_uvit_forward_cached_masks(h, x, noise_levels, out, batch, live_frames, nullptr, stream);
}

int dfot_uvit_forward_cached_masks(dfot_uvit_t h, const float* x, const float* noise_levels, float* out, int batch, const uint8_t* live_frames,
                                   const uint8_t* fresh_frames, void* stream) {
  DFOT_REQUIRE(h && x && noise_levels && out, DFOT_ERR_ARG, "forward: null argument");
  DFOT_REQUIRE(!fresh_frames || h->last_batch == batch, DFOT_ERR_STATE,
               "forward: frozen frames need the previous forward of this handle to have run the same batch (%d, now %d)", h->last_batch, batch);
  DFOT_REQUIRE(!fresh_frames || live_frames, DFOT_ERR_ARG, "forward: frozen frames must also be dead frames (live_frames is null)");
  DFOT_REQUIRE(!h->posefree, DFOT_ERR_STATE, "forward_cached: a pose-free handle (dfot_uvit3d_create) runs through dfot_uvit3d_forward");
  DFOT_REQUIRE(h->finalized, DFOT_ERR_STATE, "forward: weights not finalized");
  DFOT_REQUIRE(batch > 0 && batch == h->cond_batch, DFOT_ERR_STATE,
               "forward_cached: batch %d does not match the cached conditions (%d)", batch, h->cond_batch);
  hipStream_t s = (hipStream_t)stream;
  const dfot_uvit_config& c = h->cfg;
  const int bt = batch * h->T, e = h->E;
  int rc = 0;
  if ((rc = launch_noise_emb(noise_levels, h->ne_freqs, h->ne_phases, h->ne_w1, h->ne_b1, h->ne_w2, h->ne_b2, h->nhid,
                             h->nemb, bt, c.noise_dim, e, s)))
    return rc;
  return forward_from_emb(h, x, out, batch, live_frames, fresh_frames, s);
}

}

static int forward_from_emb(dfot_uvit_s* h, const float* x, float* out, int batch, const uint8_t* live_frames, const uint8_t* fresh_frames,
                            hipStream_t s) {
  const dfot_uvit_config& c = h->cfg;
  const int bt = batch * h->T, e = h->E;
  int rc = 0;
  if ((rc = launch_film_vec(h->film_table, h->film_chunks, h->nemb, h->sv, bt, e, s))) return rc;
  if ((rc = launch_embed_input_bf16(x, h->ein_w, h->ein_b, h->XB[0], bt, c.resolution, c.in_channels, h->ch[0], s))) return rc;
  h->gn1_nblk = 0;
  for (int l = 0; l < 4; ++l) h->xin[l] = h->X[l];
  h->xin_bf[0] = true;
  h->xin_bf[1] = h->xin_bf[2] = h->xin_bf[3] = false;

  if (fresh_frames && (h->gemm_variant != GEMM_AUTO || (h->r[2] * h->r[2]) % 512 != 0)) fresh_frames = nullptr;
  for (int l = 0; l < 2; ++l) {
    for (const ResW& w : h->down_res[l])
      if ((rc = run_res_block(h, w, l, bt, s, fresh_frames))) return rc;
    if ((rc = run_down(h, l, bt, s, fresh_frames))) return rc;
  }
  h->pend_bias = nullptr;
  for (const TrW& w : h->down_tr)
    if ((rc = run_tr_block(h, w, 2, batch, s))) return rc;
  if ((rc = flush_pending(h, s))) return rc;
  if ((rc = run_down(h, 2, bt, s))) return rc;
  for (const TrW& w : h->mid_tr)
    if ((rc = run_tr_block(h, w, 3, batch, s))) return rc;
  if ((rc = flush_pending(h, s))) return rc;
  if ((rc = run_up(h, 2, bt, s))) return rc;
  for (const TrW& w : h->up_tr)
    if ((rc = run_tr_block(h, w, 2, batch, s))) return rc;
  if ((rc = flush_pending(h, s))) return rc;
  for (int l = 1; l >= 0; --l) {
    if ((rc = run_up(h, l, bt, s, live_frames))) return rc;
    for (const ResW& w : h->up_res[l])
      if ((rc = run_res_block(h, w, l, bt, s, live_frames))) return rc;
  }
  h->last_batch = batch;
  return launch_project_output_bf16(h->XB[0], h->pout_w, h->pout_b, out, bt, c.resolution, h->ch[0], c.in_channels, s, live_frames);
}

extern "C" {

int dfot_uvit_forward(dfot_uvit_t h, const float* x, const float* noise_levels, const float* external_cond,
                      const uint8_t* external_cond_mask, float* out, int batch, void* stream) {
  DFOT_REQUIRE(h && x && noise_levels && out, DFOT_ERR_ARG, "forward: null argument");
  int rc = dfot_uvit_set_conditions(h, external_cond, external_cond_mask, batch, stream);
  if (rc) return rc;
  return dfot_uvit_forward_cached(h, x, noise_levels, out, batch, stream);
}

int dfot_uvit3d_forward_live(dfot_uvit_t h, const float* x, const float* noise_levels, const float* external_cond,
                             const uint8_t* external_cond_mask, float* out, int batch, const uint8_t* live_frames, void* stream) {
  DFOT_REQUIRE(h && x && noise_levels && out, DFOT_ERR_ARG, "uvit3d_forward: null argument");
  DFOT_REQUIRE(h->posefree, DFOT_ERR_STATE, "uvit3d_forward: the handle is a pose model (dfot_uvit_create); call dfot_uvit_forward");
  DFOT_REQUIRE(h->finalized, DFOT_ERR_STATE, "uvit3d_forward: weights not finalized");
  DFOT_REQUIRE(batch > 0 && batch <= h->max_batch, DFOT_ERR_STATE, "uvit3d_forward: batch %d exceeds reserved %d", batch, h->max_batch);
  DFOT_REQUIRE(!external_cond || h->act_dim > 0, DFOT_ERR_ARG,
               "uvit3d_forward: external_cond given, but the model was built with cond_dim 0 (no external_cond_embedding)");
  hipStream_t s = (hipStream_t)stream;
  const uint8_t* mask = (external_cond && h->act_dropout) ? external_cond_mask : nullptr;
  int rc = launch_uvit3d_emb(noise_levels, h->ne_freqs, h->ne_phases, h->ne_w1, h->ne_b1, h->ne_w2, h->ne_b2, external_cond, mask, h->ac_w1,
                             h->ac_b1, h->ac_w2, h->ac_b2, h->nemb, batch * h->T, h->cfg.noise_dim, h->act_dim, h->E, h->T, s);
  if (rc) return rc;
  h->have_mask = false;
  return forward_from_emb(h, x, out, batch, live_frames, nullptr, s);
}

int dfot_uvit3d_forward(dfot_uvit_t h, const float* x, const float* noise_levels, const float* external_cond,
                        const uint8_t* external_cond_mask, float* out, int batch, void* stream) {
  return dfot_uvit3d_forward_live(h, x, noise_levels, external_cond, external_cond_mask, out, batch, nullptr, stream);
}

int dfot_op_gn_film_silu(const void* h, const float* stats, const float* gamma, const float* beta, const void* fcache, const float* sv,
                         const uint8_t* cond_mask, void* out, int bt, int pixels, int c, int tokens, void* stream) {
  DFOT_REQUIRE(h && stats && gamma && beta && sv && out, DFOT_ERR_ARG, "op_gn_film_silu: null argument");
  DFOT_REQUIRE(bt > 0 && pixels > 0 && tokens > 0 && c > 0 && c % 32 == 0, DFOT_ERR_SHAPE,
               "op_gn_film_silu: bt %d, pixels %d, tokens %d must be positive and channels %d a multiple of 32", bt, pixels, tokens, c);
  return launch_gn_film_silu((const bf16*)h, stats, gamma, beta, (const bf16*)fcache, sv, cond_mask, (bf16*)out, bt, pixels, c, tokens,
                             (hipStream_t)stream);
}
int dfot_op_rms_film(const void* x, const float* w, const void* fcache, const float* sv, const uint8_t* cond_mask, void* out, int64_t m,
                     int c, int rows_per_bt, int tokens, float eps, void* stream) {
  DFOT_REQUIRE(x && w && sv && out, DFOT_ERR_ARG, "op_rms_film: null argument");
  DFOT_REQUIRE(m > 0 && rows_per_bt > 0 && tokens > 0 && c > 0 && c % 32 == 0 && m % rows_per_bt == 0, DFOT_ERR_SHAPE,
               "op_rms_film: rows %ld must be a positive multiple of rows_per_bt %d, channels %d a multiple of 32", (long)m, rows_per_bt, c);
  return launch_rms_film_bf16((const bf16*)x, w, (const bf16*)fcache, sv, cond_mask, (bf16*)out, (long)m, c, rows_per_bt, tokens, eps,
                              (hipStream_t)stream);
}

int dfot_uvit_read_tap(dfot_uvit_t h, const char* name, float* out, size_t capacity, void* stream) {
  DFOT_REQUIRE(h && name && out, DFOT_ERR_ARG, "read_tap: null argument");
  DFOT_REQUIRE(h->last_batch > 0, DFOT_ERR_STATE, "read_tap: no forward has run");
  hipStream_t s = (hipStream_t)stream;
  const int bt = h->last_batch * h->T;
  if (!strcmp(name, "nemb")) {
    const size_t need = (size_t)bt * h->E;
    DFOT_REQUIRE(capacity >= need, DFOT_ERR_SHAPE, "read_tap: need %zu floats, got %zu", need, capacity);
    return copy_f32(out, h->nemb, need, s);
  }
  DFOT_REQUIRE(!(h->posefree && !strcmp(name, "pose_emb0")), DFOT_ERR_NAME, "read_tap: a pose-free handle has no tap 'pose_emb0'");
  auto pixels = [&](int l) { return h->r[l] * h->r[l]; };
// ... 143 lines not shown
```

### diffusion-forcing-transformer_amd/sampler.py

```python
from __future__ import annotations

from dataclasses import dataclass, field
from typing import Callable, Dict, List, Optional, Tuple

import numpy as np
import torch

from . import capi, parallel
from .diffusion import DiffusionConfig, Schedule, denoising_loss, masked_mean
from .guidance import HistoryGuidance


@dataclass
class SamplerConfig:
    x_shape: Tuple[int, int, int] = (3, 256, 256)
    max_tokens: int = 8
    diffusion: DiffusionConfig = field(default_factory=DiffusionConfig)
    scheduling_matrix: str = "full_sequence"
    is_full_sequence: bool = False
    prediction_guidance: Dict = field(default_factory=lambda: {"name": "conditional"})
    interpolation_guidance: Dict = field(default_factory=lambda: {"name": "conditional"})
    keyframe_density: Optional[float] = None
    sliding_context_len: Optional[int] = None
    interpolation_max_batch_size: Optional[int] = None
    refinement_sampling: Optional[Dict] = None
    camera_pose_normalize_by: str = "first"
    camera_pose_bound: Optional[float] = None
    external_cond_type: str = "action"
    external_cond_dim: int = 0
    external_cond_processing: Optional[str] = None
    attention_map_steps: Tuple[int, ...] = ()


NoiseFn = Callable[[str, tuple], torch.Tensor]


def device_noise_fn(generator: Optional[torch.Generator] = None, clip: float = 20.0) -> NoiseFn:
    def fn(tag: str, shape: tuple) -> torch.Tensor:
        return torch.randn(shape, device="cuda", generator=generator).clamp_(-clip, clip)
    return fn


class DFoTVideoPoseSampler:
    def __init__(self, cfg: SamplerConfig, backbone, noise_fn: Optional[NoiseFn] = None):
        self.cfg = cfg
        self.model = backbone
        self.schedule = Schedule(cfg.diffusion)
        self.noise_fn = noise_fn or device_noise_fn(clip=cfg.diffusion.clip_noise)
        self.timesteps = cfg.diffusion.timesteps
        self.sampling_timesteps = cfg.diffusion.sampling_timesteps
        self.max_tokens = cfg.max_tokens
        self.x_shape = tuple(cfg.x_shape)
        self.trace: List[dict] = []
        self.window_forwards = 0
        self.shard_windows = False
        self.branch_parallel = False
        self._branch_split_active = False
        self.device = "cuda"
        self.dry_run = False
        self.use_graph = True
        self.skip_frozen_frames = True
        self.skip_dead_frames = True
        self.graph_replays = 0
        self.graph_captures = 0
        self._graphs: Dict[tuple, dict] = {}
        self._graphs_generation = 0
        self.attention_maps: Dict[int, dict] = {}
        if cfg.diffusion.sampling_timesteps > cfg.diffusion.timesteps:
            raise ValueError("sampling_timesteps must be <= timesteps")

    @torch.no_grad()
    def _process_conditions(self, conditions: Optional[torch.Tensor], noise_levels=None) -> Optional[torch.Tensor]:
        if conditions is None:
            return None
        if conditions.shape[-1] != 16:
            raise ValueError(f"raw camera poses must have 16 values per frame, got {conditions.shape[-1]}")
        cfg = self.cfg
        if cfg.camera_pose_normalize_by not in ("first", "mean"):
            raise ValueError(f"Unknown camera pose normalization method: {cfg.camera_pose_normalize_by}")
        interp = None
        if noise_levels is not None and getattr(self, "_interpolate_masked_poses", False):
            interp = np.asarray(noise_levels.detach().cpu().numpy() if torch.is_tensor(noise_levels) else noise_levels) == self.timesteps - 1
        if cfg.camera_pose_normalize_by == "first" and cfg.camera_pose_bound is None and interp is None:
            return torch.ops.dfot.ray_encoding(conditions, int(self.x_shape[-1]))
        from . import pose
        world = pose.normalize_poses(conditions.detach().float().cpu().numpy(), cfg.camera_pose_normalize_by, cfg.camera_pose_bound, interp)
        return torch.ops.dfot.ray_encoding(torch.from_numpy(world), int(self.x_shape[-1]), True)

    def _select_conditions(self, conditions: Optional[torch.Tensor], index) -> Optional[torch.Tensor]:
        return None if conditions is None else conditions[:, index]

    def _padded_conditions(self, conditions: Optional[torch.Tensor], index) -> Optional[torch.Tensor]:
        return None if conditions is None else self._pad_to_max_tokens(conditions[:, index])

    def _window_conditions(self, conditions: Optional[torch.Tensor]) -> Optional[torch.Tensor]:
        return self._process_conditions(conditions)

    def _check_conditions(self, conditions: Optional[torch.Tensor], length: int) -> None:
        pass

    _static_graph_cond = False

    @torch.no_grad()
    def denoising_loss(self, xs: torch.Tensor, conditions: Optional[torch.Tensor], t: torch.Tensor,
                       noise: Optional[torch.Tensor] = None, masks: Optional[torch.Tensor] = None):
        if noise is None:
            noise = self.noise_fn("train", tuple(xs.shape))
        _, per_token, x_pred, _ = denoising_loss(self.cfg.diffusion, lambda x_t, lv: self.model(x_t, lv, self._process_conditions(conditions), None),
                                                 xs, t, noise, want_x_pred=True)
        loss, per_token = masked_mean(per_token, masks)
        return x_pred, loss, per_token

    @torch.no_grad()
    def discrete_denoising_loss(self, xs: torch.Tensor, k: torch.Tensor, noise: Optional[torch.Tensor] = None,
                                masks: Optional[torch.Tensor] = None, loss_weighting: Optional[Dict] = None):
        if self.cfg.diffusion.is_continuous:
            raise ValueError("discrete_denoising_loss needs DiffusionConfig(is_continuous=False)")
        if noise is None:
            noise = self.noise_fn("train", tuple(xs.shape))
        _, per_token, x_pred, _ = denoising_loss(self.schedule, lambda x_k, lv: self.model(x_k, lv, None, None), xs, k, noise,
                                                 loss_weighting=loss_weighting, want_x_pred=True)
        loss, per_token = masked_mean(per_token, masks)
        return x_pred, loss, per_token

    def _normalize_x(self, xs: torch.Tensor, mean, std) -> torch.Tensor:
        m = torch.as_tensor(mean, dtype=xs.dtype, device=xs.device).view(-1, 1, 1)
        s = torch.as_tensor(std, dtype=xs.dtype, device=xs.device).view(-1, 1, 1)
        return (xs - m) / s

    def _unnormalize_x(self, xs: torch.Tensor, mean, std) -> torch.Tensor:
        m = torch.as_tensor(mean, dtype=xs.dtype, device=xs.device).view(-1, 1, 1)
        s = torch.as_tensor(std, dtype=xs.dtype, device=xs.device).view(-1, 1, 1)
        return xs * s + m

    def _pad_to_max_tokens(self, y: Optional[torch.Tensor]) -> Optional[torch.Tensor]:
        if y is None or y.shape[1] >= self.max_tokens:
            return y
        tail = y[:, -1:].expand(-1, self.max_tokens - y.shape[1], *y.shape[2:])
        return torch.cat([y, tail], dim=1)

    @torch.no_grad()
    def _sample_sequence(self, batch_size: int, length: Optional[int] = None, context: Optional[torch.Tensor] = None,
                         context_mask: Optional[torch.Tensor] = None, conditions: Optional[torch.Tensor] = None,
                         history_guidance: Optional[HistoryGuidance] = None, _refine: Optional[Tuple[int, int]] = None,
                         **_) -> Tuple[torch.Tensor, None]:
# ... 111 lines not shown
                if need or strict:
                    noise = self.noise_fn("q_sample", (bh, horizon, *x_shape)).to(device=dev, dtype=torch.float32)
                    if g > 1:
                        noise = noise.repeat_interleave(g, dim=0)
                if strict or p_["excl"] is not None:
                    fresh = self.noise_fn("excluded", (bh, g, horizon, *x_shape))
                    if p_["excl"] is not None:
                        fresh = fresh.to(device=dev, dtype=torch.float32).reshape(bm, horizon, *x_shape)
                        em = torch.from_numpy(p_["excl"]).to(dev).view(bm, horizon, *([1] * len(x_shape)))
                        noise = torch.where(em, fresh, noise if noise is not None else torch.zeros_like(fresh))
            return None if noise is None else noise.contiguous().view(bm, horizon, *x_shape)

        split_nfe = set()
        if self._branch_split_active:
            world_n = parallel.world_info()[0]
            for n_ in sorted({p_["nfe"] for p_ in plans if not p_.get("renoise")}):
                if n_ > 1 and world_n > 1 and world_n % n_ == 0:
                    parallel.branch_group(n_)
                    split_nfe.add(n_)
        if self.dry_run:
            for p_ in plans:
                if p_["nfe"] in split_nfe:
                    hb = parallel.world_info()[1] % p_["nfe"]
                    got = parallel.exchange_branches(torch.full((batch_size, 1), float(hb)), p_["nfe"])
                    if not torch.equal(got.view(batch_size, p_["nfe"]), torch.arange(p_["nfe"], dtype=got.dtype).repeat(batch_size, 1)):
                        raise RuntimeError("branch exchange returned the branches out of (sample, branch) order")
                    self.branch_exchanges = getattr(self, "branch_exchanges", 0) + 1
                if p_.get("renoise"):
                    self.noise_fn("renoise", (batch_size, horizon, *x_shape))
                    continue
                draw_noise(p_)
                if strict or p_["sigma"] is not None:
                    self.noise_fn("ddim", (p_["bm"], horizon, *x_shape))
                    if _refine is not None:
                        self.noise_fn("refine_context", (batch_size, horizon, *x_shape))
            self.window_forwards += sum(p_["bm"] for p_ in plans if not p_.get("renoise"))
            return (xs[:, :-padding] if padding > 0 else xs), None
        flat_dev = torch.from_numpy(np.concatenate([p_["tables"].ravel() for p_ in plans])).cuda()
        gens_dev = torch.from_numpy(np.stack([p_["gen"] for p_ in plans])).cuda()
        off = 0
        cmask_cache: Dict[bytes, torch.Tensor] = {}
        weight_cache: Dict[bytes, torch.Tensor] = {}
        lives_by_nfe: Dict[int, torch.Tensor] = {}
        for i, p_ in enumerate(plans):
            n = p_["tables"].size
            p_["tables_dev"] = flat_dev[off:off + n].view(8, p_["bm"], horizon)
            off += n
            p_["gen_dev"] = gens_dev[i]
            if p_.get("renoise"):
                continue
            if p_["nfe"] not in lives_by_nfe:
                lives_by_nfe[p_["nfe"]] = gens_dev if p_["nfe"] == 1 else gens_dev.repeat_interleave(p_["nfe"], dim=1)
            p_["live_dev"] = lives_by_nfe[p_["nfe"]][i]
            wsrc = p_["plan"].weights if p_["plan"].tok_weights is None else p_["plan"].tok_weights
            wkey = wsrc.tobytes()
            if wkey not in weight_cache:
                weight_cache[wkey] = torch.from_numpy(np.ascontiguousarray(wsrc, dtype=np.float32)).cuda()
            p_["weights_dev"] = weight_cache[wkey]
            p_["tokw"] = p_["plan"].tok_weights is not None
            p_["sigma_dev"] = None if p_["sigma"] is None else torch.from_numpy(p_["sigma"]).cuda()
            p_["cmask_dev"] = None
            if p_["cmask"] is not None:
                ckey = p_["cmask"].tobytes()
                if ckey not in cmask_cache:
                    cmask_cache[ckey] = torch.from_numpy(p_["cmask"]).cuda()
                p_["cmask_dev"] = cmask_cache[ckey]

        cond_full = None if pose_interp else self._window_conditions(conditions)
        cond_rep, cond_nfe = None, 0
        if pose_interp:
            by_mask: Dict[bytes, torch.Tensor] = {}
            self._interpolate_masked_poses = True
            try:
                for p_ in plans:
                    if p_.get("renoise"):
                        continue
                    lv = p_["plan"].levels.reshape(p_["bm"], horizon)
                    key = (lv == self.timesteps - 1).tobytes() + bytes([p_["nfe"]])
                    if key not in by_mask:
                        by_mask[key] = self._process_conditions(conditions.repeat_interleave(p_["nfe"], dim=0), lv)
                    p_["cond"] = by_mask[key]
            finally:
                self._interpolate_masked_poses = False
        fresh_dev = torch.from_numpy(np.concatenate([a.ravel() for a in self._fresh_flags(plans, batch_size, horizon)])).cuda()
        foff = 0
        for p_ in plans:
            p_["fresh_dev"] = fresh_dev[foff:foff + p_["bm"] * horizon].view(p_["bm"], horizon)
            foff += p_["bm"] * horizon
        xs = xs.contiguous()
        s = capi.stream_ptr
        branch_cache: Dict[tuple, tuple] = {}

        skip_dead = self.skip_dead_frames and hasattr(self.model, "live_frames")
        skip_frozen = skip_dead and self.skip_frozen_frames and hasattr(self.model, "fresh_frames")

        map_steps = set(int(i) for i in (getattr(cfg, "attention_map_steps", None) or ()))
        collect_at: Optional[int] = None
        if map_steps and not self.dry_run:
            if not hasattr(self.model, "capture_attention"):
                raise NotImplementedError(f"attention_map_steps: {type(self.model).__name__} has no attention-map capture (DiT3D backbones only)")
            self.attention_maps = {}

        def step(p_, xs, noise, tables, gen_dev, xs_next=None, live_dev=None, fresh_dev=None):
            nonlocal cond_rep, cond_nfe
            nfe, bm = p_["nfe"], p_["bm"]
            x_in = torch.empty(bm, horizon, *x_shape, device="cuda", dtype=torch.float32)
            capi.check(capi.lib.dfot_hg_prepare(capi.ptr(xs), capi.ptr(noise), capi.ptr(tables[0]), capi.ptr(tables[1]),
                                                capi.ptr(x_in), batch_size, nfe, horizon, f, s()))
            if cond_full is not None and cond_nfe != nfe:
                cond_rep = cond_full if nfe == 1 else cond_full.repeat_interleave(nfe, dim=0)
                cond_nfe = nfe
            if "cond" in p_:
                cond_rep = p_["cond"]
            lvl = tables[7] if cfg.diffusion.is_continuous else tables[7].to(torch.int32)
            world, rank = parallel.world_info()
            if nfe in split_nfe:
                hb = rank % nfe
                key = (id(cond_rep), id(p_["cmask_dev"]), hb)
                if key not in branch_cache:
                    c_h = None if cond_rep is None else cond_rep.view(batch_size, nfe, *cond_rep.shape[1:])[:, hb].contiguous()
                    m_h = None if p_["cmask_dev"] is None else p_["cmask_dev"].view(batch_size, nfe)[:, hb].contiguous()
                    branch_cache[key] = (c_h, m_h, cond_rep, p_["cmask_dev"])
                c_h, m_h = branch_cache[key][:2]
                x_h = x_in.view(batch_size, nfe, horizon, *x_shape)[:, hb].contiguous()
                l_h = lvl.view(batch_size, nfe, horizon)[:, hb].contiguous()
                if skip_dead:
                    self.model.live_frames = gen_dev
                try:
                    v = parallel.exchange_branches(self.model(x_h, l_h, c_h, m_h), nfe)
                    self.branch_exchanges = getattr(self, "branch_exchanges", 0) + 1
                finally:
                    if skip_dead:
                        self.model.live_frames = None
            elif rg > 0:
                v = self._reconstruction_guided_v(x_in, lvl, cond_rep, p_["cmask_dev"], tables, gen_dev, rg_ctx, rg, nfe)
            else:
                if skip_dead:
                    self.model.live_frames = live_dev if live_dev is not None else p_["live_dev"]
                if skip_frozen:
                    self.model.fresh_frames = fresh_dev if fresh_dev is not None else p_["fresh_dev"]
                try:
                    v = self.model(x_in, lvl, cond_rep, p_["cmask_dev"])
                finally:
                    if skip_dead:
                        self.model.live_frames = None
                    if skip_frozen:
                        self.model.fresh_frames = None
            if collect_at is not None:
                self.attention_maps[collect_at] = {"noise_levels": lvl.clone(), **self.model.attention_maps()}
            step_noise = None
            if strict or p_["sigma"] is not None:
                step_noise = self.noise_fn("ddim", (bm, horizon, *x_shape))
            if xs_next is None:
                xs_next = torch.empty_like(xs)
            compose = capi.lib.dfot_ddim_compose_tokw if p_["tokw"] else capi.lib.dfot_ddim_compose
            capi.check(compose(capi.ptr(xs), capi.ptr(x_in), capi.ptr(v), capi.ptr(tables[2]),
                                                  capi.ptr(tables[3]), capi.ptr(tables[4]), capi.ptr(tables[5]),
                                                  capi.ptr(tables[6]), capi.ptr(p_["weights_dev"]), capi.ptr(gen_dev),
                                                  capi.ptr(xs_next), batch_size, nfe, horizon, f, s()))
            if p_["sigma"] is not None:
                nz = step_noise.to(device="cuda", dtype=torch.float32).clamp(-cfg.diffusion.clip_noise, cfg.diffusion.clip_noise).contiguous()
                capi.check(capi.lib.dfot_ddim_noise(capi.ptr(nz), capi.ptr(p_["sigma_dev"]), capi.ptr(p_["weights_dev"]), capi.ptr(gen_dev),
                                                    capi.ptr(xs_next), batch_size, nfe, horizon, f, int(p_["tokw"]), s()))
            return xs_next

        def renoise(p_, xs):
            noise = self.noise_fn("renoise", (batch_size, horizon, *x_shape)).to(device="cuda", dtype=torch.float32)
            noise = noise.clamp(-cfg.diffusion.clip_noise, cfg.diffusion.clip_noise).contiguous()
            out = torch.empty_like(xs)
            capi.check(capi.lib.dfot_hg_prepare(capi.ptr(xs), capi.ptr(noise), capi.ptr(p_["tables_dev"][0]), capi.ptr(p_["tables_dev"][1]),
                                                capi.ptr(out), batch_size, 1, horizon, f, s()))
            return out

        if _refine is not None:
            for p_ in plans:
                if p_.get("renoise"):
                    xs = renoise(p_, xs)
                    continue
                xs = step(p_, xs, draw_noise(p_), p_["tables_dev"], p_["gen_dev"])
                if strict:
                    self.noise_fn("refine_context", (batch_size, horizon, *x_shape))
            self.window_forwards += sum(p_["bm"] for p_ in plans if not p_.get("renoise"))
            return (xs[:, :-padding] if padding > 0 else xs), None
        uniform = all(p_["bm"] == plans[0]["bm"] and p_["cmask_dev"] is plans[0]["cmask_dev"]
                      and p_["weights_dev"] is plans[0]["weights_dev"] and p_.get("cond") is plans[0].get("cond") for p_ in plans)
        hook = getattr(self, "step_hook", None)
        collecting = bool(map_steps) and not self.dry_run
        if (self.use_graph and uniform and not strict and len(plans) > 2 and all(p_["sigma"] is None for p_ in plans) and not self._branch_split_active
                and rg == 0 and hook is None and not collecting):
            if self._static_graph_cond and cond_full is not None:
                nfe0 = plans[0]["nfe"]
                plans[0]["cond_src"] = cond_full if nfe0 == 1 else cond_full.repeat_interleave(nfe0, dim=0)
            xs = self._run_steps_graph(plans, xs, draw_noise, step, flat_dev, gens_dev, horizon)
        else:
            own_capture = collecting and not self.model.capturing_attention
            if own_capture:
                self.model.capture_attention()
            try:
                for i, p_ in enumerate(plans):
                    collect_at = i if collecting and i in map_steps else None
                    xs = step(p_, xs, draw_noise(p_), p_["tables_dev"], p_["gen_dev"])
                    if hook is not None:
                        hook(i, xs)
            finally:
                collect_at = None
                if own_capture:
                    self.model.capture_attention(False)
        self.window_forwards += sum(p_["bm"] for p_ in plans)
        if padding > 0:
            xs = xs[:, :-padding]
        return xs, None

    @torch.no_grad()
    def _sample_sequence_refine(self, batch_size: int, goback_length: int, n_goback: int, length: Optional[int] = None,
                                context: Optional[torch.Tensor] = None, context_mask: Optional[torch.Tensor] = None,
                                conditions: Optional[torch.Tensor] = None, history_guidance: Optional[HistoryGuidance] = None,
                                **_) -> Tuple[torch.Tensor, None]:
        return self._sample_sequence(batch_size, length=length, context=context, context_mask=context_mask, conditions=conditions,
                                     history_guidance=history_guidance, _refine=(int(goback_length), int(n_goback)))

    def _window_sampler(self):
        return self._sample_sequence

    def _reconstruction_guided_v(self, x_in, lvl, cond, cmask, tables, gen_dev, ctx, rg: float, nfe: int):
        if nfe != 1:
            raise ValueError("reconstruction guidance needs one-branch history guidance (the reference's loss compares the "
                             "(B * NFE, ...) prediction with the (B, ...) context)")
        if self.cfg.diffusion.objective != "pred_v":
            raise ValueError("reconstruction guidance is implemented for the v objective")
        nd = x_in.ndim
        ext = lambda a: a.reshape(*a.shape, *([1] * (nd - a.ndim)))
        sa, s1 = ext(tables[2]), ext(tables[3])
        with torch.enable_grad():
            x = x_in.detach().requires_grad_(True)
            v = self.model(x, lvl, cond, cmask)
            pred_x0 = sa * x - s1 * v
            cm = ext((gen_dev == 0).to(torch.float32))
            loss = torch.sum((pred_x0 - ctx) ** 2 * sa * cm / cm.sum(dim=1, keepdim=True).clamp(min=1))
            grad = torch.nan_to_num(-torch.autograd.grad(-rg * 0.5 * loss, x)[0], nan=0.0)
        an, cn = ext(tables[4]), ext(tables[5])
        scale = torch.where(sa > 0, s1 / sa.clamp(min=1e-30), torch.where(an > 0, -cn / an.clamp(min=1e-30), torch.zeros_like(sa)))
        return (v.detach() + scale * grad).contiguous()

    @staticmethod
    def _fresh_flags(plans, batch_size: int, horizon: int):
        out, prev = [], None
        for p_ in plans:
            fresh = np.ones((p_["bm"], horizon), np.uint8)
            if p_.get("renoise"):
                out.append(fresh)
                prev = None
                continue
            if (prev is not None and prev["bm"] == p_["bm"] and prev["nfe"] == p_["nfe"] and prev.get("cond") is p_.get("cond")
                    and ((prev["cmask"] is None and p_["cmask"] is None)
                         or (prev["cmask"] is not None and p_["cmask"] is not None and np.array_equal(prev["cmask"], p_["cmask"])))):
                a, b = prev["tables"], p_["tables"]
                same_in = (a[0] == 1) & (a[1] == 0) & (b[0] == 1) & (b[1] == 0) & (a[7] == b[7])
                untouched = np.repeat(prev["gen"].reshape(batch_size, horizon) == 0, p_["nfe"], axis=0)
                fresh = np.where(same_in & untouched, 0, 1).astype(np.uint8)
            out.append(fresh)
            prev = p_
        return out

    def _run_steps_graph(self, plans, xs, draw_noise, step, flat_dev, gens_dev, horizon):
        p0 = plans[0]
        bm, n_steps, nfe = p0["bm"], len(plans), p0["nfe"]
        need_noise = any(p_["need_noise"] for p_ in plans)
        self.model.reserve(bm)
        if hasattr(self.model, "sync_weights"):
            self.model.sync_weights()
        gen = getattr(self.model, "reserve_generation", 0)
        if gen != self._graphs_generation:
            self._graphs.clear()
            self._graphs_generation = gen
        cond_src = p0.get("cond_src")
        key = (bm, n_steps, nfe, horizon, tuple(xs.shape), need_noise, None if p0["cmask"] is None else p0["cmask"].tobytes(),
               id(self.model), None if cond_src is None else (tuple(cond_src.shape), cond_src.dtype))
        ent = self._graphs.get(key)
        if ent is None:
            ent = dict(tables=torch.empty(n_steps, 8, bm, horizon, device="cuda", dtype=torch.float32),
                       gens=torch.empty_like(gens_dev), weights=torch.empty_like(p0["weights_dev"]),
                       lives=torch.empty(n_steps, bm, horizon, device="cuda", dtype=torch.uint8),
                       fresh=torch.empty(n_steps, bm, horizon, device="cuda", dtype=torch.uint8),
                       noise=torch.empty(n_steps, bm, *xs.shape[1:], device="cuda") if need_noise else None,
                       xs=torch.empty_like(xs), out=None, graph=None,
                       cond=None if cond_src is None else torch.empty_like(cond_src),
                       cmask=p0["cmask_dev"].clone() if self._static_graph_cond and p0["cmask_dev"] is not None else None)
        ent["tables"].copy_(flat_dev.view(n_steps, 8, bm, horizon))
        ent["gens"].copy_(gens_dev)
        ent["lives"].copy_(gens_dev if nfe == 1 else gens_dev.repeat_interleave(nfe, dim=1))
        ent["fresh"].copy_(torch.stack([p_["fresh_dev"] for p_ in plans]))
        ent["weights"].copy_(p0["weights_dev"])
        if need_noise:
            for i, p_ in enumerate(plans):
                if p_["need_noise"]:
                    ent["noise"][i].copy_(draw_noise(p_))
                else:
                    ent["noise"][i].zero_()
        p_static = dict(p0, weights_dev=ent["weights"])
        if ent["cmask"] is not None:
            p_static["cmask_dev"] = ent["cmask"]
        if cond_src is not None:
            ent["cond"].copy_(cond_src)
            p_static["cond"] = ent["cond"]
        ent["xs"].copy_(step(p_static, xs, None if not need_noise else ent["noise"][0], ent["tables"][0], ent["gens"][0], live_dev=ent["lives"][0],
                            fresh_dev=ent["fresh"][0]))
        if ent["graph"] is None:
            torch.cuda.synchronize()
            graph = torch.cuda.CUDAGraph()
            with torch.cuda.graph(graph, capture_error_mode="thread_local"):
                x = ent["xs"]
                for i in range(1, n_steps):
                    x = step(p_static, x, ent["noise"][i] if need_noise else None, ent["tables"][i], ent["gens"][i], live_dev=ent["lives"][i],
                             fresh_dev=ent["fresh"][i])
                ent["out"] = x
            ent["graph"] = graph
            if len(self._graphs) >= 4:
                self._graphs.pop(next(iter(self._graphs)))
            self._graphs[key] = ent
            self.graph_captures += 1
        ent["graph"].replay()
        self.graph_replays += n_steps - 1
        return ent["out"].clone()

    @torch.no_grad()
    def _predict_sequence(self, context: torch.Tensor, length: Optional[int] = None,
                          conditions: Optional[torch.Tensor] = None, history_guidance: Optional[HistoryGuidance] = None,
                          sliding_context_len: Optional[int] = None, **_) -> Tuple[torch.Tensor, None]:
        mt = self.max_tokens
        if length is None:
            length = mt
        if sliding_context_len is None:
            if mt < length:
                raise ValueError("when length > max_tokens, sliding_context_len must be specified.")
            sliding_context_len = mt - 1
        if sliding_context_len == -1:
            sliding_context_len = mt - 1
        batch_size, gt_len = context.shape[:2]
        if sliding_context_len < gt_len:
            raise ValueError("sliding_context_len is expected to be >= length of initial context,"
                             f"got {sliding_context_len}. If you are trying to use max context, "
                             "consider specifying sliding_context_len=-1.")
        xs = context.to(device=self.device, dtype=torch.float32)
        cur = gt_len
        n_window = 0
        while cur < length:
            c = min(sliding_context_len, cur)
            h = min(length - cur, mt - c)
            window = torch.cat([xs[:, -c:], xs.new_zeros(batch_size, h, *self.x_shape)], 1)
            generated = cur - max(cur - c, gt_len)
            cmask = torch.ones(batch_size, c, dtype=torch.long)
            if generated > 0:
                cmask[:, -generated:] = 2
            cmask = torch.cat([cmask, torch.zeros(batch_size, h, dtype=torch.long)], 1)
            cond = self._select_conditions(conditions, slice(cur - c, cur - c + mt))
            if hasattr(self.noise_fn, "set_windows"):
                self.noise_fn.set_windows([n_window])
            n_window += 1
            new, _ = self._window_sampler()(batch_size, length=c + h, context=window, context_mask=cmask,
                                           conditions=cond, history_guidance=history_guidance)
            xs = torch.cat([xs, new[:, -h:]], 1)
            cur = xs.shape[1]
        return xs, None

    def _interpolation_plan(self, known: np.ndarray) -> List[List[np.ndarray]]:
        mt = self.max_tokens
        known = known.copy()
        plan: List[List[np.ndarray]] = []
        while not known.all():
            keys = np.where(known)[0]
            stage: List[np.ndarray] = []
            chunk: Optional[np.ndarray] = None
            for left, right in zip(keys[:-1], keys[1:]):
                left, right = int(left), int(right)
                if chunk is not None:
                    if len(chunk) + right - left <= mt:
                        chunk = np.concatenate([chunk, np.arange(left + 1, right + 1)])
                        continue
                    stage.append(chunk)
                    chunk = None
                if right - left == 1:
                    continue
                if right - left >= mt - 1:
                    stage.append(torch.linspace(left, right, mt).round().long().numpy())
                else:
                    chunk = np.arange(left, right + 1)
            if chunk is not None:
                stage.append(chunk)
            for w in stage:
                known[w] = True
            plan.append(stage)
        return plan

    @torch.no_grad()
    def _interpolate_videos(self, context: torch.Tensor, context_mask: Optional[torch.Tensor] = None,
                            conditions: Optional[torch.Tensor] = None, **_) -> torch.Tensor:
        cfg = self.cfg
# ... 145 lines not shown
```

### include/dfot_hip.h

```cpp
#ifndef DFOT_HIP_H_
#define DFOT_HIP_H_

#include <stddef.h>
#include <stdint.h>

#ifdef __cplusplus
extern "C" {
#endif

enum {
  DFOT_OK = 0,
  DFOT_ERR_ARG = 1,
  DFOT_ERR_SHAPE = 2,
  DFOT_ERR_HIP = 3,
  DFOT_ERR_STATE = 4,
  DFOT_ERR_NAME = 5
};

typedef struct dfot_uvit_s* dfot_uvit_t;

typedef struct {
  int32_t channels[4];
  int32_t emb_channels;
  int32_t num_updown_blocks[3];
  int32_t num_mid_blocks;
  int32_t num_heads;
  int32_t in_channels;
  int32_t resolution;
  int32_t max_tokens;
  int32_t cond_dim;
  int32_t noise_dim;
  float rope_theta;
  float eps;
} dfot_uvit_config;

const char* dfot_last_error(void);
int dfot_version(void);

int dfot_uvit_create(const dfot_uvit_config* cfg, dfot_uvit_t* out);
int dfot_uvit_destroy(dfot_uvit_t h);
int dfot_uvit_num_params(dfot_uvit_t h);
const char* dfot_uvit_param_name(dfot_uvit_t h, int index);
int dfot_uvit_param_shape(dfot_uvit_t h, int index, int64_t shape[4], int* ndim);
int dfot_uvit_load_weight(dfot_uvit_t h, const char* name, const float* data, const int64_t* shape, int ndim,
                          void* stream);
int dfot_uvit_finalize(dfot_uvit_t h, void* stream);
int dfot_uvit_reserve(dfot_uvit_t h, int max_batch);
size_t dfot_uvit_workspace_bytes(dfot_uvit_t h);
int dfot_uvit_set_option(dfot_uvit_t h, const char* key, int value);
int dfot_uvit_query(dfot_uvit_t h, const char* key, double* value);
int dfot_uvit_attn_timing(dfot_uvit_t h, double* total_ms, int64_t* launches);

int dfot_uvit_forward(dfot_uvit_t h, const float* x, const float* noise_levels, const float* external_cond,
                      const uint8_t* external_cond_mask, float* out, int batch, void* stream);
int dfot_uvit_set_conditions(dfot_uvit_t h, const float* external_cond, const uint8_t* external_cond_mask, int batch,
                             void* stream);
int dfot_uvit_forward_cached(dfot_uvit_t h, const float* x, const float* noise_levels, float* out, int batch,
                             void* stream);
int dfot_uvit_forward_cached_live(dfot_uvit_t h, const float* x, const float* noise_levels, float* out, int batch,
                                  const uint8_t* live_frames, void* stream);
int dfot_uvit_forward_cached_masks(dfot_uvit_t h, const float* x, const float* noise_levels, float* out, int batch,
                                   const uint8_t* live_frames, const uint8_t* fresh_frames, void* stream);
int dfot_uvit_read_tap(dfot_uvit_t h, const char* name, float* out, size_t capacity_floats, void* stream);

typedef struct {
  int32_t channels[4];
  int32_t emb_channels;
  int32_t num_updown_blocks[3];
  int32_t num_mid_blocks;
  int32_t num_heads;
  int32_t in_channels;
  int32_t resolution;
  int32_t max_tokens;
  int32_t cond_dim;
  int32_t noise_dim;
  float rope_theta;
  float eps;
  int32_t cond_dropout;
} dfot_uvit3d_config;
int dfot_uvit3d_create(const dfot_uvit3d_config* cfg, dfot_uvit_t* out);
int64_t dfot_uvit3d_config_bytes(void);
int dfot_uvit3d_forward(dfot_uvit_t h, const float* x, const float* noise_levels, const float* external_cond,
                        const uint8_t* external_cond_mask, float* out, int batch, void* stream);
int dfot_uvit3d_forward_live(dfot_uvit_t h, const float* x, const float* noise_levels, const float* external_cond,
                             const uint8_t* external_cond_mask, float* out, int batch, const uint8_t* live_frames, void* stream);
int dfot_op_gn_film_silu(const void* h, const float* stats, const float* gamma, const float* beta, const void* fcache, const float* sv,
                         const uint8_t* cond_mask, void* out, int bt, int pixels, int c, int tokens, void* stream);
int dfot_op_rms_film(const void* x, const float* w, const void* fcache, const float* sv, const uint8_t* cond_mask, void* out, int64_t m,
                     int c, int rows_per_bt, int tokens, float eps, void* stream);

typedef struct dfot_dit_s* dfot_dit_t;

typedef struct {
  int32_t hidden_size;
  int32_t depth;
  int32_t num_heads;
  int32_t patch_size;
  int32_t in_channels;
  int32_t height;
  int32_t width;
  int32_t max_tokens;
  int32_t mlp_hidden;
  int32_t noise_dim;
  int32_t timesteps;
  float rope_theta;
  float eps;
  int32_t variant;
  int32_t embed_col_dim;
  int32_t num_col_heads;
  int32_t num_row_heads;
  int32_t temporal_mlp_hidden;
  int32_t use_bias;
  int32_t cond_type;
  int32_t cond_dim;
  int32_t num_classes;
  int32_t cond_dropout;
  int32_t use_temporal_rope;
} dfot_dit_config;
enum { DFOT_COND_NONE = 0, DFOT_COND_ACTION = 1, DFOT_COND_LABEL = 2 };

typedef struct {
  dfot_dit_config base;
  int32_t fourier_noise;
} dfot_dit_config_f;

int dfot_dit_create(const dfot_dit_config* cfg, dfot_dit_t* out);
int dfot_dit_create_f(const dfot_dit_config_f* cfg, dfot_dit_t* out);
int dfot_dit_destroy(dfot_dit_t h);
int dfot_dit_num_params(dfot_dit_t h);
const char* dfot_dit_param_name(dfot_dit_t h, int index);
int dfot_dit_param_shape(dfot_dit_t h, int index, int64_t shape[4], int* ndim);
int dfot_dit_load_weight(dfot_dit_t h, const char* name, const float* data, const int64_t* shape, int ndim, void* stream);
int dfot_dit_finalize(dfot_dit_t h, void* stream);
int dfot_dit_reserve(dfot_dit_t h, int max_batch);
size_t dfot_dit_workspace_bytes(dfot_dit_t h);
int dfot_dit_set_option(dfot_dit_t h, const char* key, int value);
int dfot_dit_attn_timing(dfot_dit_t h, double* total_ms, int64_t* launches);
int dfot_dit_forward(dfot_dit_t h, const float* x, const int32_t* noise_levels, float* out, int batch, int tokens,
                     void* stream);
int dfot_dit_forward_cond(dfot_dit_t h, const float* x, const int32_t* noise_levels, const float* cond, const int32_t* labels,
                          const uint8_t* cond_mask, float* out, int batch, int tokens, void* stream);
int dfot_dit_forward_f(dfot_dit_t h, const float* x, const float* noise_levels, const float* cond, const int32_t* labels,
                       const uint8_t* cond_mask, float* out, int batch, int tokens, void* stream);
int dfot_dit_read_tap(dfot_dit_t h, const char* name, float* out, size_t capacity_floats, void* stream);
int dfot_op_dit_final_layer(const float* x, const float* table, const int32_t* levels, int64_t ldt, int64_t off, const float* w, const float* b,
// ... 274 lines not shown
```

Baseline: 10.31.

## Share down-path ResBlock work across identical guidance-branch frames

```diff
diff --git a/diffusion-forcing-transformer_amd/backbone.py b/diffusion-forcing-transformer_amd/backbone.py
--- a/diffusion-forcing-transformer_amd/backbone.py
+++ b/diffusion-forcing-transformer_amd/backbone.py
@@ -4,6 +4,7 @@
 import math
 from typing import Dict, Optional, Sequence, Tuple
 
+import numpy as np
 import torch
 from torch import nn
 
@@ -18,6 +19,26 @@
 
 class _Node(nn.Module):
     """Anonymous container so that dotted reference key names map onto a module tree."""
+
+
+def down_plan(twin: np.ndarray, fresh: Optional[np.ndarray]):
+    tw = np.asarray(twin).reshape(-1).astype(np.int64)
+    idx = np.arange(tw.size)
+    if ((tw < 0) | (tw > idx)).any():
+        i = int(np.argmax((tw < 0) | (tw > idx)))
+        raise ValueError(f"twin_frames: image {i} names image {int(tw[i])}: a twin is an EARLIER image of the batch (src < dst)")
+    if (tw[tw] != tw).any():
+        i = int(np.argmax(tw[tw] != tw))
+        raise ValueError(f"twin_frames: image {i} names image {int(tw[i])}, which is itself a duplicate (of {int(tw[tw[i]])})")
+    need = tw == idx
+    if fresh is not None:
+        need &= np.asarray(fresh).reshape(-1) != 0
+    dst = idx[tw != idx]
+    pairs = np.ascontiguousarray(np.stack([dst, tw[dst]], axis=1), dtype=np.int32)
+    if not need.any():
+        return 0, int(tw.size), pairs, True
+    lo, hi = int(idx[need][0]), int(idx[need][-1]) + 1
+    return lo, hi, pairs, bool((~need[lo:hi]).any())
 
 
 class UViT3DPose(nn.Module):
@@ -80,7 +101,10 @@
         self._trainer_sig = None
         self.live_frames = None
         self.fresh_frames = None
+        self.twin_frames = None
+        self.fresh_frames_host = None
         self._fresh_key = None
+        self._last_batch = 0
         self._train_stamp = 0
         self._dropout_generator: Optional[torch.Generator] = None
 
@@ -336,13 +360,38 @@
             if tuple(fresh.shape) != (b, self.temporal_length) or fresh.dtype != torch.uint8 or not fresh.is_contiguous():
                 raise ValueError(f"fresh_frames must be a contiguous uint8 tensor of shape {(b, self.temporal_length)}")
             capi.require_device(dev, fresh_frames=fresh)
-            if key != self._fresh_key:
+            if key != self._fresh_key and self.twin_frames is None:
                 fresh = None
-        capi.check(capi.lib.dfot_uvit_forward_cached_masks(self._handle, capi.ptr(xf, torch.float32, "x"),
-                                                           capi.ptr(kf, torch.float32, "noise_levels"), capi.ptr(out), b,
-                                                           capi.ptr(live, torch.uint8, "live_frames"),
-                                                           capi.ptr(fresh, torch.uint8, "fresh_frames"), capi.stream_ptr()))
+        twin = self.twin_frames
+        if twin is None:
+            capi.check(capi.lib.dfot_uvit_forward_cached_masks(self._handle, capi.ptr(xf, torch.float32, "x"),
+                                                               capi.ptr(kf, torch.float32, "noise_levels"), capi.ptr(out), b,
+                                                               capi.ptr(live, torch.uint8, "live_frames"),
+                                                               capi.ptr(fresh, torch.uint8, "fresh_frames"), capi.stream_ptr()))
+        else:
+            twin = np.asarray(twin)
+            if tuple(twin.shape) != (b, self.temporal_length) or twin.dtype != np.int32:
+                raise ValueError(f"twin_frames must be an int32 host array of shape {(b, self.temporal_length)}")
+            fresh_host = None
+            if fresh is not None:
+                fresh_host = self.fresh_frames_host
+                if fresh_host is None:
+                    if torch.cuda.is_current_stream_capturing():
+                        raise RuntimeError("twin_frames with fresh_frames under stream capture needs fresh_frames_host (no read-back while capturing)")
+                    fresh_host = fresh.cpu().numpy()
+                if tuple(np.shape(fresh_host)) != (b, self.temporal_length):
+                    raise ValueError(f"fresh_frames_host must have shape {(b, self.temporal_length)}")
+            if fresh is not None and key != self._fresh_key and (
+                    self._last_batch != b or (np.asarray(fresh_host)[twin == np.arange(twin.size).reshape(twin.shape)] == 0).any()):
+                fresh = fresh_host = None
+            lo, hi, pairs, holes = down_plan(twin, fresh_host)
+            capi.check(capi.lib.dfot_uvit_forward_cached_shared(self._handle, capi.ptr(xf, torch.float32, "x"),
+                                                                capi.ptr(kf, torch.float32, "noise_levels"), capi.ptr(out), b,
+                                                                capi.ptr(live, torch.uint8, "live_frames"),
+                                                                capi.ptr(fresh if holes else None, torch.uint8, "fresh_frames"), lo, hi,
+                                                                pairs.ctypes.data if len(pairs) else None, len(pairs), capi.stream_ptr()))
         self._fresh_key = key
+        self._last_batch = b
         return out.to(x.dtype)
 
     def read_tap(self, name: str, channels: int, level: int, batch: int) -> torch.Tensor:
diff --git a/diffusion-forcing-transformer_amd/capi.py b/diffusion-forcing-transformer_amd/capi.py
--- a/diffusion-forcing-transformer_amd/capi.py
+++ b/diffusion-forcing-transformer_amd/capi.py
@@ -99,6 +99,7 @@
     "dfot_uvit_forward_cached": (_I, [_P, _P, _P, _P, _I, _P]),
     "dfot_uvit_forward_cached_live": (_I, [_P, _P, _P, _P, _I, _P, _P]),
     "dfot_uvit_forward_cached_masks": (_I, [_P, _P, _P, _P, _I, _P, _P, _P]),
+    "dfot_uvit_forward_cached_shared": (_I, [_P, _P, _P, _P, _I, _P, _P, _I, _I, _P, _I, _P]),
     "dfot_uvit_read_tap": (_I, [_P, C.c_char_p, _P, C.c_size_t, _P]),
     "dfot_uvit3d_create": (_I, [C.POINTER(UViT3DConfig), C.POINTER(_P)]),
     "dfot_uvit3d_config_bytes": (_L, []),
diff --git a/diffusion-forcing-transformer_amd/csrc/gemm.h b/diffusion-forcing-transformer_amd/csrc/gemm.h
--- a/diffusion-forcing-transformer_amd/csrc/gemm.h
+++ b/diffusion-forcing-transformer_amd/csrc/gemm.h
@@ -12,6 +12,7 @@
   const bf16* W = nullptr;
   long ldw = 0;
   int M = 0, N = 0, K = 0;
+  int pick_m = 0;
   int H = 0, Wd = 0, Cin = 0;
   const bf16* zeros = nullptr;
   const uint8_t* live = nullptr;
diff --git a/diffusion-forcing-transformer_amd/csrc/gemm.hip b/diffusion-forcing-transformer_amd/csrc/gemm.hip
--- a/diffusion-forcing-transformer_amd/csrc/gemm.hip
+++ b/diffusion-forcing-transformer_amd/csrc/gemm.hip
@@ -847,7 +847,7 @@
 
 int launch_gemm(int amode, int epi, int variant, const GemmArgs& g, hipStream_t stream) {
   DFOT_REQUIRE(g.A && g.W, DFOT_ERR_ARG, "gemm: null operand");
-  if (variant == GEMM_AUTO) variant = gemm_pick_variant(amode, g.M, g.N, g.K, epi == E_F32 && !g.gn_part);
+  if (variant == GEMM_AUTO) variant = gemm_pick_variant(amode, g.pick_m > 0 ? g.pick_m : g.M, g.N, g.K, epi == E_F32 && !g.gn_part);
   if (variant == GEMM_DMA_128_KS2 && epi == E_QKV) variant = GEMM_DMA_128;
   if (variant == GEMM_DMA_128x192 && epi == E_QKV) variant = GEMM_DMA_128;
   if (variant == GEMM_DMA_256x192 && epi == E_QKV && g.d != 64) variant = GEMM_DMA_256x256;
diff --git a/diffusion-forcing-transformer_amd/csrc/kernels.h b/diffusion-forcing-transformer_amd/csrc/kernels.h
--- a/diffusion-forcing-transformer_amd/csrc/kernels.h
+++ b/diffusion-forcing-transformer_amd/csrc/kernels.h
@@ -81,6 +81,15 @@
 int launch_f32_to_bf16(const float* src, bf16* dst, long n, hipStream_t s);
 int launch_bf16_to_f32(const bf16* src, float* dst, long n, hipStream_t s);
 int launch_equal_bits(const void* a, const void* b, long bytes, int* differs, hipStream_t s);
+constexpr int ROWCOPY_MAX_TENSORS = 4, ROWCOPY_MAX_PAIRS = 64;
+struct RowCopyArgs {
+  char* base[ROWCOPY_MAX_TENSORS];
+  long image_bytes[ROWCOPY_MAX_TENSORS];
+  int pieces[ROWCOPY_MAX_TENSORS];
+  int ntensors;
+  int dst[ROWCOPY_MAX_PAIRS], src[ROWCOPY_MAX_PAIRS];
+};
+int launch_copy_image_rows(char* const* base, const long* image_bytes, int ntensors, const int* pairs, int npairs, int images, hipStream_t s);
 int launch_pack_rows(const float* src, bf16* dst, const int* map, int rows, int k, int kpad, long ldd, int col0,
                      hipStream_t s);
 int launch_pack_conv3(const float* src, bf16* dst, int co, int ci, hipStream_t s);
diff --git a/diffusion-forcing-transformer_amd/csrc/kernels.hip b/diffusion-forcing-transformer_amd/csrc/kernels.hip
--- a/diffusion-forcing-transformer_amd/csrc/kernels.hip
+++ b/diffusion-forcing-transformer_amd/csrc/kernels.hip
@@ -1547,6 +1547,56 @@
   if ((al & 3) == 0) return launch_equal_bits_t<unsigned int>(a, b, bytes, differs, s);
   return launch_equal_bits_t<uint8_t>(a, b, bytes, differs, s);
 }
+
+constexpr int ROWCOPY_BLOCK = 256, ROWCOPY_UNROLL = 4;
+constexpr long ROWCOPY_CHUNK = (long)ROWCOPY_BLOCK * ROWCOPY_UNROLL * 16;
+
+__global__ __launch_bounds__(ROWCOPY_BLOCK) void copy_image_rows_kernel(RowCopyArgs a) {
+  const int dst = a.dst[blockIdx.y], src = a.src[blockIdx.y];
+  int piece = blockIdx.x, t = 0;
+  while (t + 1 < a.ntensors && piece >= a.pieces[t]) piece -= a.pieces[t++];
+  const long units = a.image_bytes[t] >> 4;
+  const uint4v* __restrict__ from = reinterpret_cast<const uint4v*>(a.base[t] + (long)src * a.image_bytes[t]);
+  uint4v* __restrict__ to = reinterpret_cast<uint4v*>(a.base[t] + (long)dst * a.image_bytes[t]);
+  const long u0 = (long)piece * (ROWCOPY_BLOCK * ROWCOPY_UNROLL) + threadIdx.x;
+  uint4v v[ROWCOPY_UNROLL];
+#pragma unroll
+  for (int j = 0; j < ROWCOPY_UNROLL; ++j)
+    if (u0 + j * ROWCOPY_BLOCK < units) v[j] = from[u0 + j * ROWCOPY_BLOCK];
+#pragma unroll
+  for (int j = 0; j < ROWCOPY_UNROLL; ++j)
+    if (u0 + j * ROWCOPY_BLOCK < units) to[u0 + j * ROWCOPY_BLOCK] = v[j];
+}
+
+int launch_copy_image_rows(char* const* base, const long* image_bytes, int ntensors, const int* pairs, int npairs, int images, hipStream_t s) {
+  DFOT_REQUIRE(base && image_bytes && ntensors > 0 && ntensors <= ROWCOPY_MAX_TENSORS && npairs >= 0 && (npairs == 0 || pairs), DFOT_ERR_ARG,
+               "copy_image_rows: bad argument (%d tensors, %d pairs)", ntensors, npairs);
+  RowCopyArgs a{};
+  a.ntensors = ntensors;
+  long pieces = 0;
+  for (int t = 0; t < ntensors; ++t) {
+    DFOT_REQUIRE(base[t] && ((uintptr_t)base[t] & 15) == 0 && image_bytes[t] > 0 && image_bytes[t] % 16 == 0, DFOT_ERR_ARG,
+                 "copy_image_rows: tensor %d needs a 16-byte aligned base and a multiple of 16 bytes per image (%ld)", t, image_bytes[t]);
+    a.base[t] = base[t];
+    a.image_bytes[t] = image_bytes[t];
+    a.pieces[t] = (int)cdiv(image_bytes[t], ROWCOPY_CHUNK);
+    pieces += a.pieces[t];
+  }
+  DFOT_REQUIRE(pieces < (1L << 31), DFOT_ERR_SHAPE, "copy_image_rows: images too large");
+  for (int i = 0; i < npairs; ++i)
+    DFOT_REQUIRE(pairs[2 * i] >= 0 && pairs[2 * i] < images && pairs[2 * i + 1] >= 0 && pairs[2 * i + 1] < images && pairs[2 * i] != pairs[2 * i + 1],
+                 DFOT_ERR_ARG, "copy_image_rows: pair %d = (%d, %d) outside the %d images, or an image onto itself", i, pairs[2 * i], pairs[2 * i + 1], images);
+  for (int p0 = 0; p0 < npairs; p0 += ROWCOPY_MAX_PAIRS) {
+    const int n = npairs - p0 < ROWCOPY_MAX_PAIRS ? npairs - p0 : ROWCOPY_MAX_PAIRS;
+    for (int i = 0; i < n; ++i) {
+      a.dst[i] = pairs[2 * (p0 + i)];
+      a.src[i] = pairs[2 * (p0 + i) + 1];
+    }
+    hipLaunchKernelGGL(copy_image_rows_kernel, dim3((unsigned)pieces, (unsigned)n), dim3(ROWCOPY_BLOCK), 0, s, a);
+    DFOT_CHECK_HIP(hipGetLastError());
+  }
+  return DFOT_OK;
+}
 }
 
 extern "C" int dfot_op_equal_bits(const void* a, const void* b, int64_t bytes, int32_t* differs, void* stream) {
diff --git a/diffusion-forcing-transformer_amd/csrc/uvit.hip b/diffusion-forcing-transformer_amd/csrc/uvit.hip
--- a/diffusion-forcing-transformer_amd/csrc/uvit.hip
+++ b/diffusion-forcing-transformer_amd/csrc/uvit.hip
@@ -362,37 +362,45 @@
   if (i < n) o[i] = a[i] + b[i];
 }
 
-static int run_res_block(dfot_uvit_s* h, const ResW& w, int lvl, int bt, hipStream_t s, const uint8_t* live = nullptr) {
+struct SubBatch {
+  int lo = 0, full = 0;
+};
+static int run_res_block(dfot_uvit_s* h, const ResW& w, int lvl, int bt, hipStream_t s, const uint8_t* live = nullptr, SubBatch sub = SubBatch{}) {
   const int c = w.c, rr = h->r[lvl], pix = rr * rr;
   const int m = bt * pix;
   const int slots = pix / 64;
-  bf16* xb = h->XB[lvl];
+  const long act0 = (long)sub.lo * pix * c;
+  const int pick_m = sub.full ? sub.full * pix : 0;
+  bf16* xb = h->XB[lvl] + act0;
+  bf16 *s1 = h->s1 + act0, *hbf = h->hbf + act0;
+  float* stats = h->gn_stats + (long)sub.lo * 64;
+  auto part = [&](float* base, int nblk) { return base + (long)sub.lo * nblk * 64; };
   int rc = 0;
   if (!h->xin_bf[lvl]) {
-    if ((rc = launch_f32_to_bf16(h->xin[lvl], xb, (long)m * c, s))) return rc;
+    if ((rc = launch_f32_to_bf16(h->xin[lvl] + act0, xb, (long)m * c, s))) return rc;
     h->xin_bf[lvl] = true;
   }
   if (h->gn1_nblk == 0) {
-    if ((rc = launch_gn_partial_bf16(xb, h->gn_partial, bt, pix, c, s))) return rc;
     h->gn1_nblk = gn_partial_blocks(pix);
-  }
-  if ((rc = launch_gn_finalize(h->gn_partial, h->gn_stats, bt, h->gn1_nblk, pix, c, h->cfg.eps, s))) return rc;
+    if ((rc = launch_gn_partial_bf16(xb, part(h->gn_partial, h->gn1_nblk), bt, pix, c, s))) return rc;
+  }
+  if ((rc = launch_gn_finalize(part(h->gn_partial, h->gn1_nblk), stats, bt, h->gn1_nblk, pix, c, h->cfg.eps, s))) return rc;
   h->gn1_nblk = 0;
-  if ((rc = launch_gn_apply_silu_bf16in(xb, h->gn_stats, w.g1, w.be1, h->s1, bt, pix, c, s, live))) return rc;
+  if ((rc = launch_gn_apply_silu_bf16in(xb, stats, w.g1, w.be1, s1, bt, pix, c, s, live))) return rc;
   GemmArgs g;
-  g.A = h->s1; g.W = w.w1; g.M = m; g.N = c; g.K = 9 * c; g.H = rr; g.Wd = rr; g.Cin = c; g.zeros = h->zeros;
-  g.bias = w.bias1; g.out_bf16 = h->hbf; g.ldo = c; g.live = live;
-  g.gn_part = h->gn_partial2; g.gn_rows_per_bt = pix; g.gn_cpg = c / 32;
+  g.A = s1; g.W = w.w1; g.M = m; g.pick_m = pick_m; g.N = c; g.K = 9 * c; g.H = rr; g.Wd = rr; g.Cin = c; g.zeros = h->zeros;
+  g.bias = w.bias1; g.out_bf16 = hbf; g.ldo = c; g.live = live;
+  g.gn_part = part(h->gn_partial2, slots); g.gn_rows_per_bt = pix; g.gn_cpg = c / 32;
   if ((rc = launch_gemm(A_CONV3, E_BF16, h->gemm_variant, g, s))) return rc;
-  if ((rc = launch_gn_finalize(h->gn_partial2, h->gn_stats, bt, slots, pix, c, h->cfg.eps, s))) return rc;
-  if ((rc = launch_gn_film_silu(h->hbf, h->gn_stats, w.g2, w.be2, w.fcache, h->sv + w.sv_off,
-                                h->have_mask ? h->cond_mask : nullptr, h->s1, bt, pix, c, h->T, s, live)))
+  if ((rc = launch_gn_finalize(g.gn_part, stats, bt, slots, pix, c, h->cfg.eps, s))) return rc;
+  if ((rc = launch_gn_film_silu(hbf, stats, w.g2, w.be2, w.fcache ? w.fcache + 2 * act0 : nullptr, h->sv + w.sv_off + (long)sub.lo * 2 * c,
+                                h->have_mask ? h->cond_mask : nullptr, s1, bt, pix, c, h->T, s, live)))
     return rc;
   GemmArgs o;
-  o.A = h->s1; o.W = w.w2; o.M = m; o.N = c; o.K = 9 * c; o.H = rr; o.Wd = rr; o.Cin = c; o.zeros = h->zeros;
+  o.A = s1; o.W = w.w2; o.M = m; o.pick_m = pick_m; o.N = c; o.K = 9 * c; o.H = rr; o.Wd = rr; o.Cin = c; o.zeros = h->zeros;
   o.bias = w.bias2; o.out_bf16 = xb; o.ldo = c; o.live = live;
   o.resid_bf = xb;
-  o.gn_part = h->gn_partial; o.gn_rows_per_bt = pix; o.gn_cpg = c / 32;
+  o.gn_part = part(h->gn_partial, slots); o.gn_rows_per_bt = pix; o.gn_cpg = c / 32;
   if ((rc = launch_gemm(A_CONV3, E_BF16, h->gemm_variant, o, s))) return rc;
   h->xin_bf[lvl] = true;
   h->gn1_nblk = slots;
@@ -497,16 +505,17 @@
 
 static int conv_between_levels(dfot_uvit_s* h, GemmArgs g, hipStream_t s) {
   const long px = (long)g.H * g.Wd;
-  if (h->gemm_variant == GEMM_AUTO && h->out_part && !g.gn_part && g.M % 256 == 0 && px % 256 == 0 && (g.N % 144 == 0 || g.N == 256) &&
-      (long)g.M * g.N < (1L << 31)) {
+  const int full_m = g.pick_m > 0 ? g.pick_m : g.M;
+  if (h->gemm_variant == GEMM_AUTO && h->out_part && !g.gn_part && full_m % 256 == 0 && g.M % 256 == 0 && px % 256 == 0 &&
+      (g.N % 144 == 0 || g.N == 256) && (long)full_m * g.N < (1L << 31)) {
     const int bn = g.N % 144 == 0 ? 144 : 256;
     const int variant = bn == 144 ? GEMM_DMA3_256x144 : GEMM_DMA_256x256;
-    const int tiles = (g.M / 256) * (g.N / bn);
+    const int tiles = (full_m / 256) * (g.N / bn);
     int ks = 1;
     while (tiles * ks * 2 <= 256 && g.K / 64 / (ks * 2) >= 16) ks *= 2;
     if (tiles * ks >= 192 && tiles * ks <= 256) {
       if (ks == 1) return launch_gemm(A_CONV3, E_F32, variant, g, s);
-      if ((size_t)ks * g.M * g.N <= h->out_part_elems) {
+      if ((size_t)ks * full_m * g.N <= h->out_part_elems) {
         GemmArgs p = g;
         float* out = g.out_f32;
         const float* bias = g.bias;
@@ -524,18 +533,22 @@
   return launch_gemm(A_CONV3, E_F32, h->gemm_variant, g, s);
 }
 
-static int run_down(dfot_uvit_s* h, int l, int bt, hipStream_t s, const uint8_t* live = nullptr) {
+static int run_down(dfot_uvit_s* h, int l, int bt, hipStream_t s, const uint8_t* live = nullptr, SubBatch sub = SubBatch{}) {
   const int rr = h->r[l], cin = h->ch[l], cout = h->ch[l + 1];
+  const long pin = (long)rr * rr, pout = pin / 4;
+  bf16* s1 = h->s1 + sub.lo * pout * cin;
   int rc = 0;
-  if ((rc = h->xin_bf[l] ? launch_pool2_bf16_bf16in(h->XB[l], h->s1, bt, rr, rr, cin, s) : launch_pool2_bf16(h->xin[l], h->s1, bt, rr, rr, cin, s)))
+  if ((rc = h->xin_bf[l] ? launch_pool2_bf16_bf16in(h->XB[l] + sub.lo * pin * cin, s1, bt, rr, rr, cin, s)
+                         : launch_pool2_bf16(h->xin[l] + sub.lo * pin * cin, s1, bt, rr, rr, cin, s)))
     return rc;
   GemmArgs g;
-  g.A = h->s1; g.W = h->down_conv[l].w; g.M = bt * (rr / 2) * (rr / 2); g.N = cout; g.K = 9 * cin; g.H = rr / 2; g.Wd = rr / 2;
-  g.Cin = cin; g.zeros = h->zeros; g.bias = h->down_conv[l].b; g.out_f32 = h->HSA[l]; g.ldo = cout;
+  g.A = s1; g.W = h->down_conv[l].w; g.M = bt * (rr / 2) * (rr / 2); g.N = cout; g.K = 9 * cin; g.H = rr / 2; g.Wd = rr / 2;
+  g.pick_m = sub.full ? sub.full * (rr / 2) * (rr / 2) : 0;
+  g.Cin = cin; g.zeros = h->zeros; g.bias = h->down_conv[l].b; g.out_f32 = h->HSA[l] + sub.lo * pout * cout; g.ldo = cout;
   g.live = live;
   const bool next_is_res = l + 1 < 2;
   if (next_is_res) {
-    g.gn_part = h->gn_partial; g.gn_rows_per_bt = (rr / 2) * (rr / 2); g.gn_cpg = cout / 32;
+    g.gn_part = h->gn_partial + sub.lo * (pout / 64) * 64; g.gn_rows_per_bt = (rr / 2) * (rr / 2); g.gn_cpg = cout / 32;
   }
   if ((rc = conv_between_levels(h, g, s))) return rc;
   h->gn1_nblk = next_is_res ? g.gn_rows_per_bt / 64 : 0;
@@ -566,8 +579,13 @@
 
 }
 
+struct DownPlan {
+  int lo, hi;
+  const int32_t* pairs;
+  int npairs;
+};
 static int forward_from_emb(dfot_uvit_s* h, const float* x, float* out, int batch, const uint8_t* live_frames, const uint8_t* fresh_frames,
-                            hipStream_t s);
+                            hipStream_t s, const DownPlan* plan = nullptr);
 
 extern "C" {
 
@@ -907,7 +925,31 @@
 
 int dfot_uvit_forward_cached_masks(dfot_uvit_t h, const float* x, const float* noise_levels, float* out, int batch, const uint8_t* live_frames,
                                    const uint8_t* fresh_frames, void* stream) {
+  return dfot_uvit_forward_cached_shared(h, x, noise_levels, out, batch, live_frames, fresh_frames, 0, h ? batch * h->T : 0, nullptr, 0, stream);
+}
+
+int dfot_uvit_forward_cached_shared(dfot_uvit_t h, const float* x, const float* noise_levels, float* out, int batch, const uint8_t* live_frames,
+                                    const uint8_t* fresh_frames, int lo, int hi, const int32_t* pairs, int npairs, void* stream) {
   DFOT_REQUIRE(h && x && noise_levels && out, DFOT_ERR_ARG, "forward: null argument");
+  {
+    const int n = batch * h->T;
+    DFOT_REQUIRE(batch > 0 && 0 <= lo && lo < hi && hi <= n, DFOT_ERR_ARG, "forward: image range [%d, %d) outside the %d images of the batch", lo, hi, n);
+    DFOT_REQUIRE(npairs >= 0 && (npairs == 0 || pairs), DFOT_ERR_ARG, "forward: %d image pairs without a list", npairs);
+    std::vector<uint8_t> is_dst((size_t)n, 0);
+    for (int i = 0; i < npairs; ++i) {
+      const int dst = pairs[2 * i], src = pairs[2 * i + 1];
+      DFOT_REQUIRE(0 <= src && src < dst && dst < n, DFOT_ERR_ARG, "forward: pair %d copies image %d onto %d: need 0 <= src < dst < %d", i, src, dst, n);
+      DFOT_REQUIRE(!is_dst[dst], DFOT_ERR_ARG, "forward: image %d is the destination of two pairs", dst);
+      is_dst[dst] = 1;
+    }
+    bool kept = false;
+    for (int i = 0; i < npairs; ++i)
+      DFOT_REQUIRE(!is_dst[pairs[2 * i + 1]], DFOT_ERR_ARG, "forward: source image %d of pair %d is itself a destination", pairs[2 * i + 1], i);
+    for (int i = 0; i < n; ++i) kept = kept || ((i < lo || i >= hi) && !is_dst[i]);
+    DFOT_REQUIRE(!kept || h->last_batch == batch, DFOT_ERR_STATE,
+                 "forward: images outside the range need the previous forward of this handle to have run the same batch (%d, now %d)", h->last_batch, batch);
+    DFOT_REQUIRE(!kept || live_frames, DFOT_ERR_ARG, "forward: images outside the range must also be dead frames (live_frames is null)");
+  }
   DFOT_REQUIRE(!fresh_frames || h->last_batch == batch, DFOT_ERR_STATE,
                "forward: frozen frames need the previous forward of this handle to have run the same batch (%d, now %d)", h->last_batch, batch);
   DFOT_REQUIRE(!fresh_frames || live_frames, DFOT_ERR_ARG, "forward: frozen frames must also be dead frames (live_frames is null)");
@@ -922,28 +964,54 @@
   if ((rc = launch_noise_emb(noise_levels, h->ne_freqs, h->ne_phases, h->ne_w1, h->ne_b1, h->ne_w2, h->ne_b2, h->nhid,
                              h->nemb, bt, c.noise_dim, e, s)))
     return rc;
-  return forward_from_emb(h, x, out, batch, live_frames, fresh_frames, s);
+  const DownPlan plan{lo, hi, pairs, npairs};
+  return forward_from_emb(h, x, out, batch, live_frames, fresh_frames, s, (lo > 0 || hi < bt || npairs > 0) ? &plan : nullptr);
 }
 
 }
 
 static int forward_from_emb(dfot_uvit_s* h, const float* x, float* out, int batch, const uint8_t* live_frames, const uint8_t* fresh_frames,
-                            hipStream_t s) {
+                            hipStream_t s, const DownPlan* plan) {
   const dfot_uvit_config& c = h->cfg;
   const int bt = batch * h->T, e = h->E;
   int rc = 0;
   if ((rc = launch_film_vec(h->film_table, h->film_chunks, h->nemb, h->sv, bt, e, s))) return rc;
-  if ((rc = launch_embed_input_bf16(x, h->ein_w, h->ein_b, h->XB[0], bt, c.resolution, c.in_channels, h->ch[0], s))) return rc;
   h->gn1_nblk = 0;
   for (int l = 0; l < 4; ++l) h->xin[l] = h->X[l];
   h->xin_bf[0] = true;
   h->xin_bf[1] = h->xin_bf[2] = h->xin_bf[3] = false;
 
-  if (fresh_frames && (h->gemm_variant != GEMM_AUTO || (h->r[2] * h->r[2]) % 512 != 0)) fresh_frames = nullptr;
+  const bool whole_tiles = h->gemm_variant == GEMM_AUTO && (h->r[2] * h->r[2]) % 512 == 0;
+  int lo = 0, hi = bt;
+  if (plan && !(fresh_frames && !whole_tiles) && !(h->have_mask && !h->posefree)) {
+    lo = plan->lo;
+    hi = plan->hi;
+    int gran = 512, rows = h->r[2] * h->r[2];
+    while (rows % 2 == 0 && gran > 1) { rows /= 2; gran /= 2; }
+    const int n = (hi - lo + gran - 1) / gran * gran;
+    if (n >= bt) { lo = 0; hi = bt; }
+    else { hi = std::min(bt, lo + n); lo = hi - n; }
+  }
+  if (fresh_frames && !whole_tiles) fresh_frames = nullptr;
+  const int nb = hi - lo;
+  const SubBatch sub{lo, nb < bt ? bt : 0};
+  const uint8_t* fresh = fresh_frames ? fresh_frames + lo : nullptr;
+  if ((rc = launch_embed_input_bf16(x + (long)lo * c.in_channels * c.resolution * c.resolution, h->ein_w, h->ein_b,
+                                    h->XB[0] + (long)lo * h->r[0] * h->r[0] * h->ch[0], nb, c.resolution, c.in_channels, h->ch[0], s)))
+    return rc;
   for (int l = 0; l < 2; ++l) {
     for (const ResW& w : h->down_res[l])
-      if ((rc = run_res_block(h, w, l, bt, s, fresh_frames))) return rc;
-    if ((rc = run_down(h, l, bt, s, fresh_frames))) return rc;
+      if ((rc = run_res_block(h, w, l, nb, s, fresh, sub))) return rc;
+    if ((rc = run_down(h, l, nb, s, fresh, sub))) return rc;
+  }
+  if (plan && plan->npairs > 0) {
+    char* const base[4] = {(char*)h->XB[0], (char*)h->XB[1], (char*)h->HSA[0], (char*)h->HSA[1]};
+    long bytes[4];
+    for (int l = 0; l < 2; ++l) {
+      bytes[l] = (long)h->r[l] * h->r[l] * h->ch[l] * (long)sizeof(bf16);
+      bytes[2 + l] = (long)h->r[l + 1] * h->r[l + 1] * h->ch[l + 1] * (long)sizeof(float);
+    }
+    if ((rc = launch_copy_image_rows(base, bytes, 4, plan->pairs, plan->npairs, bt, s))) return rc;
   }
   h->pend_bias = nullptr;
   for (const TrW& w : h->down_tr)
diff --git a/diffusion-forcing-transformer_amd/sampler.py b/diffusion-forcing-transformer_amd/sampler.py
--- a/diffusion-forcing-transformer_amd/sampler.py
+++ b/diffusion-forcing-transformer_amd/sampler.py
@@ -61,6 +61,7 @@
         self.use_graph = True
         self.skip_frozen_frames = True
         self.skip_dead_frames = True
+        self.share_branch_frames = True
         self.graph_replays = 0
         self.graph_captures = 0
         self._graphs: Dict[tuple, dict] = {}
@@ -338,7 +339,14 @@
                     p_["cond"] = by_mask[key]
             finally:
                 self._interpolate_masked_poses = False
-        fresh_dev = torch.from_numpy(np.concatenate([a.ravel() for a in self._fresh_flags(plans, batch_size, horizon)])).cuda()
+        fresh_host = list(self._fresh_flags(plans, batch_size, horizon))
+        if (self.share_branch_frames and self.skip_dead_frames and self.skip_frozen_frames
+                and all(hasattr(self.model, a) for a in ("live_frames", "fresh_frames", "twin_frames"))):
+            for i, (p_, tw) in enumerate(zip(plans, self._twin_frames(plans, batch_size, horizon))):
+                if tw is not None and (tw.ravel() != np.arange(tw.size)).any():
+                    fresh_host[i] = np.where(tw != np.arange(tw.size, dtype=tw.dtype).reshape(tw.shape), 0, fresh_host[i]).astype(np.uint8)
+                    p_["twin"], p_["fresh_host"] = tw, fresh_host[i]
+        fresh_dev = torch.from_numpy(np.concatenate([a.ravel() for a in fresh_host])).cuda()
         foff = 0
         for p_ in plans:
             p_["fresh_dev"] = fresh_dev[foff:foff + p_["bm"] * horizon].view(p_["bm"], horizon)
@@ -357,8 +365,9 @@
                 raise NotImplementedError(f"attention_map_steps: {type(self.model).__name__} has no attention-map capture (DiT3D backbones only)")
             self.attention_maps = {}
 
-        def step(p_, xs, noise, tables, gen_dev, xs_next=None, live_dev=None, fresh_dev=None):
+        def step(p_, xs, noise, tables, gen_dev, xs_next=None, live_dev=None, fresh_dev=None, host_plan=None):
             nonlocal cond_rep, cond_nfe
+            host_plan = p_ if host_plan is None else host_plan
             nfe, bm = p_["nfe"], p_["bm"]
             x_in = torch.empty(bm, horizon, *x_shape, device="cuda", dtype=torch.float32)
             capi.check(capi.lib.dfot_hg_prepare(capi.ptr(xs), capi.ptr(noise), capi.ptr(tables[0]), capi.ptr(tables[1]),
@@ -395,6 +404,8 @@
                     self.model.live_frames = live_dev if live_dev is not None else p_["live_dev"]
                 if skip_frozen:
                     self.model.fresh_frames = fresh_dev if fresh_dev is not None else p_["fresh_dev"]
+                    if host_plan.get("twin") is not None:
+                        self.model.twin_frames, self.model.fresh_frames_host = host_plan["twin"], host_plan["fresh_host"]
                 try:
                     v = self.model(x_in, lvl, cond_rep, p_["cmask_dev"])
                 finally:
@@ -402,6 +413,8 @@
                         self.model.live_frames = None
                     if skip_frozen:
                         self.model.fresh_frames = None
+                        if host_plan.get("twin") is not None:
+                            self.model.twin_frames = self.model.fresh_frames_host = None
             if collect_at is not None:
                 self.attention_maps[collect_at] = {"noise_levels": lvl.clone(), **self.model.attention_maps()}
             step_noise = None
@@ -518,6 +531,25 @@
             prev = p_
         return out
 
+    @staticmethod
+    def _twin_frames(plans, batch_size: int, horizon: int):
+        out = []
+        for p_ in plans:
+            if p_.get("renoise") or p_["nfe"] < 2 or "cond" in p_:
+                out.append(None)
+                continue
+            nfe, bm, t = p_["nfe"], p_["bm"], p_["tables"]
+            plain = (t[0] == 1) & (t[1] == 0)
+            bits = np.zeros(bm, bool) if p_["cmask"] is None else np.asarray(p_["cmask"], bool)
+            own = np.arange(bm * horizon, dtype=np.int32).reshape(bm, horizon)
+            twin = own.copy()
+            for r in range(bm):
+                for r2 in range(r - r % nfe, r):
+                    same = plain[r] & plain[r2] & (t[7, r] == t[7, r2]) & (twin[r] == own[r]) & (bits[r] == bits[r2])
+                    twin[r, same] = own[r2, same]
+            out.append(twin)
+        return out
+
     def _run_steps_graph(self, plans, xs, draw_noise, step, flat_dev, gens_dev, horizon):
         p0 = plans[0]
         bm, n_steps, nfe = p0["bm"], len(plans), p0["nfe"]
@@ -531,7 +563,8 @@
             self._graphs_generation = gen
         cond_src = p0.get("cond_src")
         key = (bm, n_steps, nfe, horizon, tuple(xs.shape), need_noise, None if p0["cmask"] is None else p0["cmask"].tobytes(),
-               id(self.model), None if cond_src is None else (tuple(cond_src.shape), cond_src.dtype))
+               id(self.model), None if cond_src is None else (tuple(cond_src.shape), cond_src.dtype),
+               tuple(None if p_.get("twin") is None else (p_["twin"].tobytes(), p_["fresh_host"].tobytes()) for p_ in plans))
         ent = self._graphs.get(key)
         if ent is None:
             ent = dict(tables=torch.empty(n_steps, 8, bm, horizon, device="cuda", dtype=torch.float32),
@@ -560,7 +593,7 @@
             ent["cond"].copy_(cond_src)
             p_static["cond"] = ent["cond"]
         ent["xs"].copy_(step(p_static, xs, None if not need_noise else ent["noise"][0], ent["tables"][0], ent["gens"][0], live_dev=ent["lives"][0],
-                            fresh_dev=ent["fresh"][0]))
+                            fresh_dev=ent["fresh"][0], host_plan=plans[0]))
         if ent["graph"] is None:
             torch.cuda.synchronize()
             graph = torch.cuda.CUDAGraph()
@@ -568,7 +601,7 @@
                 x = ent["xs"]
                 for i in range(1, n_steps):
                     x = step(p_static, x, ent["noise"][i] if need_noise else None, ent["tables"][i], ent["gens"][i], live_dev=ent["lives"][i],
-                             fresh_dev=ent["fresh"][i])
+                             fresh_dev=ent["fresh"][i], host_plan=plans[i])
                 ent["out"] = x
             ent["graph"] = graph
             if len(self._graphs) >= 4:
diff --git a/include/dfot_hip.h b/include/dfot_hip.h
--- a/include/dfot_hip.h
+++ b/include/dfot_hip.h
@@ -61,6 +61,9 @@
                                   const uint8_t* live_frames, void* stream);
 int dfot_uvit_forward_cached_masks(dfot_uvit_t h, const float* x, const float* noise_levels, float* out, int batch,
                                    const uint8_t* live_frames, const uint8_t* fresh_frames, void* stream);
+int dfot_uvit_forward_cached_shared(dfot_uvit_t h, const float* x, const float* noise_levels, float* out, int batch,
+                                    const uint8_t* live_frames, const uint8_t* fresh_frames, int lo, int hi, const int32_t* pairs,
+                                    int npairs, void* stream);
 int dfot_uvit_read_tap(dfot_uvit_t h, const char* name, float* out, size_t capacity_floats, void* stream);
 
 typedef struct {
```

After: 10.31, median of 3. No clear change (+0.0%).
